# nglaze00/SCoNe_GCN

Hardware: NVIDIA B200
Metric: SCoNe train trajectories/sec (higher is better)
Workload: dtype f32

## Files before the change

### __graft_entry__.py

```python
import os
import shutil
import subprocess
import sys

ROOT = os.path.dirname(os.path.abspath(__file__))
SRC = ['scone_gcn_b200/csrc/scone_complex.cu', 'scone_gcn_b200/csrc/scone_kernels.cu', 'scone_gcn_b200/csrc/scone_model.cu',
       'scone_gcn_b200/csrc/scone_bunch.cu', 'scone_gcn_b200/csrc/scone_slab.cu', 'scone_gcn_b200/csrc/scone_rows.cu',
       'scone_gcn_b200/csrc/scone_fused.cu', 'scone_gcn_b200/csrc/scone_plan_table.cu', 'scone_gcn_b200/csrc/scone_umma.cu',
       'scone_gcn_b200/csrc/scone_dp.cu']
OUT = 'scone_gcn_b200/libscone_b200.so'
NVCC_FLAGS = ['-O3', '-std=c++17', '-gencode', 'arch=compute_100a,code=sm_100a', '-lineinfo', '-Xcompiler', '-fPIC',
              '-Iinclude']
OBJ_DIR = 'build/obj'


def _stale(out, deps):
    if not os.path.exists(out):
        return True
    t = os.path.getmtime(out)
    return any(os.path.getmtime(d) > t for d in deps)


def build(force=False):
    os.chdir(ROOT)
    deps = SRC + ['include/scone_b200.h', 'scone_gcn_b200/csrc/common.cuh', 'scone_gcn_b200/csrc/slab_common.cuh', 'scone_gcn_b200/csrc/fused.cuh']
    hdrs = ['include/scone_b200.h', 'scone_gcn_b200/csrc/common.cuh', 'scone_gcn_b200/csrc/slab_common.cuh', 'scone_gcn_b200/csrc/fused.cuh']
    if force or _stale(OUT, deps):
        nvcc = shutil.which('nvcc') or '/usr/local/cuda/bin/nvcc'
        os.makedirs(OBJ_DIR, exist_ok=True)
        objs, procs = [], []
        for src in SRC:
            obj = os.path.join(OBJ_DIR, os.path.basename(src)[:-3] + '.o')
            objs.append(obj)
            if force or _stale(obj, [src] + hdrs):
                cmd = [nvcc] + NVCC_FLAGS + ['-c', '-o', obj, src]
                print('[build]', ' '.join(cmd), flush=True)
                procs.append((cmd, subprocess.Popen(cmd)))
        for cmd, p in procs:
            if p.wait() != 0:
                raise subprocess.CalledProcessError(p.returncode, cmd)
        cmd = [nvcc, '-shared', '-gencode', 'arch=compute_100a,code=sm_100a', '-o', OUT] + objs
        print('[build]', ' '.join(cmd), flush=True)
        subprocess.check_call(cmd)
    _build_xla_ffi_shim(force)
    if ROOT not in sys.path:
        sys.path.insert(0, ROOT)
    import scone_gcn_b200
    L = scone_gcn_b200.lib()
    assert L.scone_version() == 100
    print('[build] ok:', scone_gcn_b200.library_path())


def _build_xla_ffi_shim(force=False):
    src, out = 'scone_gcn_b200/csrc/scone_xla_ffi.cc', 'scone_gcn_b200/libscone_b200_xla.so'
    inc = None
    try:
        import jaxlib
        cand = os.path.join(os.path.dirname(jaxlib.__file__), 'include')
        if os.path.exists(os.path.join(cand, 'xla', 'ffi', 'api', 'ffi.h')):
            inc = cand
    except Exception:
        pass
    cxx = shutil.which('g++') or 'g++'
    if inc is None:
        os.makedirs(OBJ_DIR, exist_ok=True)
        subprocess.check_call([cxx, '-std=c++17', '-Iinclude', '-c', '-o', os.path.join(OBJ_DIR, 'scone_xla_ffi.o'), src])
        print('[build] jax FFI shim skipped (jaxlib / xla/ffi/api/ffi.h not found); %s compile-checked' % src, flush=True)
        return
    if force or _stale(out, [src, 'include/scone_b200.h', OUT]):
        cuda_inc = os.path.join(os.environ.get('CUDA_HOME', '/usr/local/cuda'), 'include')
        cmd = [cxx, '-std=c++17', '-O2', '-shared', '-fPIC', '-Iinclude', '-I' + inc, '-I' + cuda_inc, '-o', out, src,
               '-Lscone_gcn_b200', '-lscone_b200', '-Wl,-rpath,$ORIGIN']
        print('[build]', ' '.join(cmd), flush=True)
        subprocess.check_call(cmd)


def smoke():
    os.chdir(ROOT)
    for p in (ROOT, os.path.join(ROOT, 'tests')):
        if p not in sys.path:
            sys.path.insert(0, p)
    import numpy as np
    import torch
    assert torch.cuda.is_available(), 'smoke() needs a CUDA device'
    torch.cuda.set_device(0)
    import scone_gcn_b200 as sg
    from golden_util import Dataset
    from oracle import scone_oracle as so
    ds = Dataset('dataset_small.npz')
    cx = sg.SimplicialComplex.from_simplices(ds.N, ds.edges, ds.faces, 'scone')
    net = sg.SconeModel(cx, [16, 16, 16], micro_batch=32)
    rs = np.random.RandomState(0)
    W = [0.3 * rs.randn(*s) for s in net.shapes]
    net.set_weights(W)
    ptr, fe, fv = sg.flows_to_csr(ds.flows)
    lp = net.forward(ptr, fe, fv, ds.last_nodes)
    orc = so.DenseOracle('scone', so.shift_matrices(ds.B1, ds.B2, 'scone'), ds.B1, ds.last_nodes, ds.flows, ds.targets)
    with torch.no_grad():
        ref = orc.forward(W).numpy()[:, :, 0]
    err = float(np.abs(lp - ref).max())
    assert err < 1e-5 * max(1.0, float(np.abs(ref).max())), 'log-prob mismatch vs oracle: %g' % err
    mask = ds.train_mask.astype(np.float32)
    buf = net.loss_grad(ptr, fe, fv, ds.last_nodes, ds.raw['targets_argmax'], mask)
    l_ref, g_ref = orc.loss_and_grads(W, ds.train_mask, 0.0)
    n = net.n_params
    g = net.unflatten(buf[:n] / buf[n + 1])
    gerr = max(float(np.abs(a - b).max() / max(np.abs(b).max(), 1e-30)) for a, b in zip(g, g_ref))
    assert abs(buf[n] / buf[n + 1] - l_ref) < 1e-5 * max(1.0, abs(float(l_ref))) and gerr < 1e-4, (buf[n] / buf[n + 1], l_ref, gerr)
    net.adam_step(0, 1e-3, 5e-5)
    torch.cuda.synchronize()
    print('[smoke] ok: max |dlogp| = %.2e, max rel grad err = %.2e, launches = %d'
          % (err, gerr, sg.lib().scone_launch_count()))


if __name__ == '__main__':
    {'build': build, 'smoke': smoke}[sys.argv[1] if len(sys.argv) > 1 else 'build']()
```

### scone_gcn_b200/csrc/scone_fused.cu

```cuda
#include <algorithm>
#include <cstdlib>
#include <cub/device/device_radix_sort.cuh>
#include "common.cuh"
#include "fused.cuh"

namespace {

#include "slab_common.cuh"

constexpr int kTrajThreads = 256;
constexpr int kFuMaxD = SCONE_MAX_DEGREE;
constexpr uint32_t kNoRow = 0xFFFFu;
constexpr uint32_t kFlaggedKey = 0xFFFFFFu;

template <int ACT>
__device__ __forceinline__ float fu_act(float z) {
    if (ACT == SCONE_ACT_TANH) return scone_tanh(z);
    if (ACT == SCONE_ACT_LEAKY_RELU) return z >= 0.f ? z : 0.01f * z;
    return fmaxf(z, 0.f);
}
template <int ACT>
__device__ __forceinline__ float fu_dact(float h) {
    if (ACT == SCONE_ACT_TANH) return 1.f - h * h;
    if (ACT == SCONE_ACT_LEAKY_RELU) return h >= 0.f ? 1.f : 0.01f;
    return h > 0.f ? 1.f : 0.f;
}

__device__ __forceinline__ int align2(int x) { return (x + 1) & ~1; }

struct EdgeSet {
    int* keys;
    int mask, shift;
    __device__ __forceinline__ unsigned home(int e) const { return ((unsigned)e * 2654435761u) >> shift; }
    __device__ __forceinline__ int insert(int e, bool& is_new) {
        unsigned h = home(e);
        is_new = false;
        for (int probes = 0; probes <= mask; ++probes) {
            const int old = atomicCAS(&keys[h], -1, e);
            if (old == -1) {
                is_new = true;
                return (int)h;
            }
            if (old == e) return (int)h;
            h = (h + 1) & mask;
        }
        return -1;
    }
    __device__ __forceinline__ int find(int e) const {
        unsigned h = home(e);
        int k = keys[h];
        while (k != e) {
            if (k == -1) return -1;
            h = (h + 1) & mask;
            k = keys[h];
        }
        return (int)h;
    }
};

struct FuPairs {
    int s_ptr[kFuMaxD], s_off[kFuMaxD + 1];
    __device__ __forceinline__ int setup(const int32_t* __restrict__ nbrhoods, const int32_t* __restrict__ inc_ptr, int last, bool last_ok, int D) {
        for (int j = threadIdx.x; j < D; j += blockDim.x) {
            const int nbr = last_ok ? nbrhoods[(size_t)last * D + j] : -1;
            s_ptr[j] = nbr >= 0 ? inc_ptr[nbr] : -1;
            s_off[j + 1] = nbr >= 0 ? inc_ptr[nbr + 1] - inc_ptr[nbr] : 0;
        }
        __syncthreads();
        if (threadIdx.x == 0) {
            s_off[0] = 0;
            for (int j = 0; j < D; ++j) s_off[j + 1] += s_off[j];
        }
        __syncthreads();
        return s_off[D];
    }
    __device__ __forceinline__ int slot_of(int i, int D) const {
        int j = 0;
        while (j + 1 < D && s_off[j + 1] <= i) ++j;
        return j;
    }
};

template <int THREADS>
__device__ __forceinline__ void plan_trajectory(const PlanArgs& a, const int t, unsigned char* sm) {
    constexpr int QUADS = THREADS / 4;
    const int HS = a.HS, LV = a.LV, EC = a.EC, L = a.L, D = a.D;
    int* keys = reinterpret_cast<int*>(sm);
    float* xv = reinterpret_cast<float*>(keys + HS);
    int* lvl = reinterpret_cast<int*>(xv + HS);
    uint16_t* idx0 = reinterpret_cast<uint16_t*>(lvl + HS);
    int* rowcnt = reinterpret_cast<int*>(idx0 + 3 * HS);
    int* erow = rowcnt + LV + 4;
    int* live_edge = erow + LV + 4;
    uint16_t* live = reinterpret_cast<uint16_t*>(live_edge + LV);
    uint16_t* rankA = live + LV;
    uint16_t* rankB = rankA + LV;
    uint16_t* ebuf = rankB + LV;
    __shared__ FuPairs pairs;
    __shared__ int s_nhash, s_nlive, s_ovf, s_warp[THREADS / 32];
    __shared__ unsigned s_piece;

    const int tid = threadIdx.x, lane = tid & 31, ql = tid & 3;
    const unsigned qmask = 0xFu << (lane & ~3);
    int* hdr = a.hdr + (size_t)t * kFusedHdrW;
    auto give_up = [&]() {
        if (tid == 0) {
            if (a.retry != nullptr) {
                hdr[0] = kFusedFlagRetry;
                a.retry[atomicAdd(a.n_retry, 1)] = t;
            } else {
                hdr[0] = kFusedFlagOverflow;
                *a.overflow = 1;
            }
        }
    };
    for (int i = tid; i < HS; i += THREADS) {
        keys[i] = -1;
        xv[i] = 0.f;
        lvl[i] = 0;
    }
    for (int i = tid; i < 3 * HS; i += THREADS) idx0[i] = (uint16_t)kNoRow;
    if (tid == 0) s_nhash = s_ovf = s_nlive = 0;
    const int last = a.last_nodes[t];
    const bool last_ok = last >= 0 && last < a.N;
    const int total_pairs = pairs.setup(a.nbrhoods, a.inc_ptr, last, last_ok, D);
    EdgeSet set{keys, HS - 1, a.hshift};
    const int hash_cap = (HS * 3) / 4;
    auto alloc = [&](int words) -> unsigned {
        __syncthreads();
        if (tid == 0) {
            const unsigned long long w = (unsigned long long)align2(words);
            const unsigned long long o = atomicAdd(a.bump, w);
            if (o + w > a.arena_words) {
                s_ovf = 2;
                s_piece = 0u;
            } else {
                s_piece = (unsigned)o;
            }
        }
        __syncthreads();
        return s_piece;
    };
    const int fp0 = a.traj_ptr[t], fp1 = a.traj_ptr[t + 1];

    {
        const unsigned c0 = last_ok ? a.cone_ptr[last] : 0u, c1 = last_ok ? a.cone_ptr[last + 1] : 0u;
        const int n_cone = (int)(c1 - c0);
        if (n_cone > hash_cap) {
            give_up();
            return;
        }
        for (int i = tid; i < n_cone; i += THREADS) {
            const uint32_t en = a.cone_ent[c0 + i];
            bool is_new;
            const int s = set.insert((int)(en & 0x3FFFFFFFu), is_new);
            lvl[s] = (int)(en >> 30);
        }
        if (tid == 0) s_nhash = n_cone;
    }
    __syncthreads();
    for (int p = fp0 + tid; p < fp1; p += THREADS) {
        const int eo = a.flow_edge[p];
        if (eo < 0 || eo >= a.E) continue;
        const int s = set.find(a.rank[eo]);
        if (s >= 0) xv[s] = a.flow_val[p];
    }
    __syncthreads();
    auto mark = [&](int s2, int l) {
        const int bit = 1 << (8 + l);
        const int old = atomicOr(&lvl[s2], bit);
        if (!(old & bit)) {
            const int k = atomicAdd(&s_nlive, 1);
            if (k < LV) {
                live[k] = (uint16_t)s2;
                live_edge[k] = keys[s2];
            } else {
                s_ovf = 1;
            }
        }
    };
    auto rank_live = [&](uint16_t* idx, uint16_t* byrank) -> int {
        __syncthreads();
        const int n = min(s_nlive, LV);
        for (int k = tid; k < n; k += THREADS) {
            const int e = live_edge[k];
            int r = 0;
            for (int m = 0; m < n; ++m) r += live_edge[m] < e ? 1 : 0;
            idx[live[k]] = (uint16_t)r;
            byrank[r] = live[k];
        }
        __syncthreads();
        return n;
    };

    for (int p = fp0 + (tid >> 2); p < fp1; p += QUADS) {
        const int eo = a.flow_edge[p];
        if (eo < 0 || eo >= a.E) continue;
        const int e = a.rank[eo];
        const int s = set.find(e);
        if (s < 0 || xv[s] == 0.f) continue;
        const int p1 = a.mptr[e + 1];
        for (int q = a.mptr[e] + ql; q < p1; q += 4) {
            const int s2 = set.find(a.ment[q].x);
            if (s2 >= 0 && (lvl[s2] & 0xFF) >= 1) mark(s2, 1);
        }
    }
    uint16_t *rcur = rankA, *rnext = rankB;
    int n_cur = rank_live(idx0 + 1 * HS, rcur);
    if (s_ovf) {
        give_up();
        return;
    }
    int n_l[kFusedMaxL + 1] = {0, 0, 0, 0};
    unsigned off_l1 = 0, off_f[kFusedMaxL + 1] = {0, 0, 0, 0}, off_b[kFusedMaxL + 1] = {0, 0, 0, 0};
    int tot_f[kFusedMaxL + 1] = {0, 0, 0, 0}, tot_b[kFusedMaxL + 1] = {0, 0, 0, 0};

    auto emit_program = [&](const uint16_t* byrank, int n_rows, const uint16_t* idx, int& total_out) -> unsigned {
        for (int r = tid >> 2; r < n_rows; r += QUADS) {
            const int b0 = erow[r], b1 = erow[r + 1];
            int c = 0;
            for (int i = b0 + ql; i < b1; i += 4) {
                const uint32_t s2 = ebuf[i];
                if (s2 != kNoRow && idx[s2] != (uint16_t)kNoRow) ++c;
            }
            c += __shfl_xor_sync(qmask, c, 1);
            c += __shfl_xor_sync(qmask, c, 2);
            if (ql == 0) rowcnt[r] = c;
        }
        __syncthreads();
        const int total = fused_block_scan_excl<THREADS>(rowcnt, n_rows, s_warp);
        total_out = total;
        const unsigned off = alloc(align2(n_rows + 1) + 2 * total);
        if (!s_ovf) {
            int* pdst = reinterpret_cast<int*>(a.arena + off);
            int2* edst = reinterpret_cast<int2*>(a.arena + off + align2(n_rows + 1));
            for (int r = tid; r <= n_rows; r += THREADS) pdst[r] = rowcnt[r];
            for (int r = tid >> 2; r < n_rows; r += QUADS) {
                const int e = keys[byrank[r]];
                const int p0 = a.mptr[e], b0 = erow[r], b1 = erow[r + 1];
                int base = rowcnt[r];
                for (int i0 = b0; i0 < b1; i0 += 4) {
                    const int i = i0 + ql;
                    uint32_t rr = kNoRow;
                    if (i < b1) {
                        const uint32_t s2 = ebuf[i];
                        if (s2 != kNoRow) rr = idx[s2];
                    }
                    const bool valid = rr != kNoRow;
                    const unsigned bits = (__ballot_sync(qmask, valid) >> (lane & ~3)) & 0xFu;
                    if (valid) {
                        const int2 en = a.ment[p0 + (i - b0)];
                        edst[base + __popc(bits & ((1u << ql) - 1u))] = make_int2((int)(rr | (en.x == e ? 0x80000000u : 0u)), en.y);
                    }
                    base += __popc(bits);
                }
            }
        }
        __syncthreads();
        return off;
    };

    for (int l = 1; l <= L; ++l) {
        uint16_t* idx_prev = idx0 + ((l + 2) % 3) * HS;
        uint16_t* idx_next = idx0 + ((l + 1) % 3) * HS;
        n_l[l] = n_cur;
        for (int r = tid; r < n_cur; r += THREADS) {
            const int e = keys[rcur[r]];
            rowcnt[r] = a.mptr[e + 1] - a.mptr[e];
        }
        __syncthreads();
        const int n_ent = fused_block_scan_excl<THREADS>(rowcnt, n_cur, s_warp);
        if (n_ent > EC) {
            if (tid == 0) s_ovf = 1;
            __syncthreads();
            break;
        }
        for (int r = tid; r <= n_cur; r += THREADS) erow[r] = rowcnt[r];
        __syncthreads();
        for (int r = tid >> 2; r < n_cur; r += QUADS) {
            const int e = keys[rcur[r]];
            const int p0 = a.mptr[e], b0 = erow[r], len = erow[r + 1] - b0;
            for (int i = ql; i < len; i += 4) {
                const int s2 = set.find(a.ment[p0 + i].x);
                ebuf[b0 + i] = s2 >= 0 ? (uint16_t)s2 : (uint16_t)kNoRow;
            }
        }
        __syncthreads();
        if (l == 1) {
            off_l1 = alloc(3 * n_cur);
            if (!s_ovf) {
                float* dst = reinterpret_cast<float*>(a.arena + off_l1);
                for (int r = tid >> 2; r < n_cur; r += QUADS) {
                    const int slot = rcur[r];
                    const int e = keys[slot];
                    const int p0 = a.mptr[e], b0 = erow[r], len = erow[r + 1] - b0;
                    float a1 = 0.f, a2 = 0.f;
                    for (int i = ql; i < len; i += 4) {
                        const uint32_t s2 = ebuf[b0 + i];
                        const float x = s2 != kNoRow ? xv[s2] : 0.f;
                        if (x != 0.f) {
                            const int pk = a.ment[p0 + i].y;
                            a1 = fmaf((float)(short)(pk & 0xffff), x, a1);
                            a2 = fmaf((float)(pk >> 16), x, a2);
                        }
                    }
#pragma unroll
                    for (int o = 1; o < 4; o <<= 1) {
                        a1 += __shfl_xor_sync(qmask, a1, o);
                        a2 += __shfl_xor_sync(qmask, a2, o);
                    }
                    if (ql == 0) {
                        dst[3 * r + 0] = xv[slot];
                        dst[3 * r + 1] = a1;
                        dst[3 * r + 2] = a2;
                    }
                }
            }
            __syncthreads();
        } else {
            off_f[l] = emit_program(rcur, n_cur, idx_prev, tot_f[l]);
        }
        if (l == L) break;
        if (tid == 0) s_nlive = 0;
        for (int i = tid; i < HS; i += THREADS) idx_next[i] = (uint16_t)kNoRow;
        __syncthreads();
        for (int i = tid; i < n_ent; i += THREADS) {
            const uint32_t s2 = ebuf[i];
            if (s2 != kNoRow && (lvl[s2] & 0xFF) >= l + 1) mark((int)s2, l + 1);
        }
        const int n_next = rank_live(idx_next, rnext);
        if (s_ovf) break;
        off_b[l + 1] = emit_program(rcur, n_cur, idx_next, tot_b[l + 1]);
        uint16_t* tmp = rcur; rcur = rnext; rnext = tmp;
        n_cur = n_next;
    }
    __syncthreads();
    if (s_ovf == 1) {
        give_up();
        return;
    }
    const uint16_t* idxL = idx0 + (L % 3) * HS;
    const unsigned off_ro = alloc(align2(D + 1) + 2 * total_pairs);
    if (!s_ovf) {
        int* pdst = reinterpret_cast<int*>(a.arena + off_ro);
        int2* edst = reinterpret_cast<int2*>(a.arena + off_ro + align2(D + 1));
        for (int j = tid; j <= D; j += THREADS) pdst[j] = pairs.s_off[j];
        for (int i = tid; i < total_pairs; i += THREADS) {
            const int j = pairs.slot_of(i, D);
            const int2 es = a.inc_ent[pairs.s_ptr[j] + (i - pairs.s_off[j])];
            const int s = set.find(es.x);
            const uint32_t r = s >= 0 ? (uint32_t)idxL[s] : kNoRow;
            edst[i] = make_int2((int)(r | ((uint32_t)j << 16)), es.y);
        }
    }
    __syncthreads();
    if (s_ovf) {
        if (tid == 0) {
            hdr[0] = kFusedFlagOverflow;
            *a.overflow = 1;
        }
        return;
    }
    if (tid == 0) {
        hdr[0] = 0;
        for (int l = 1; l <= kFusedMaxL; ++l) hdr[l] = l <= L ? n_l[l] : 0;
        hdr[4] = (int)off_l1;
        for (int l = 2; l <= kFusedMaxL; ++l) {
            hdr[5 + (l - 2)] = (int)off_f[l];
            hdr[7 + (l - 2)] = (int)off_b[l];
        }
        hdr[9] = (int)off_ro;
        hdr[10] = total_pairs;
        hdr[11] = s_nhash;
        hdr[12] = tot_f[2];
        hdr[13] = fp1 - fp0;
        hdr[14] = tot_f[3];
        hdr[15] = min(tot_b[2], 0xFFFF) | (min(tot_b[3], 0xFFFF) << 16);
    }
}

template <int THREADS>
__global__ void __launch_bounds__(THREADS) fused_plan_kernel(const PlanArgs a) {
    extern __shared__ __align__(16) unsigned char sm[];
    const int n_work = a.tier == 0 ? a.n_work : *a.n_in;
    for (int w = blockIdx.x; w < n_work; w += gridDim.x) {
        plan_trajectory<THREADS>(a, a.tier == 0 ? w : a.in_list[w], sm);
        __syncthreads();
    }
}

struct TrajArgs {
    const int* hdr;
    const uint32_t* arena;
    const int32_t* rows;
    const uint32_t* okeys;
    const int32_t* order;
    const float* W;
    int w_off[3 * kFusedMaxL + 1];
    int L, b, D, n_params;
    float* logprobs;
    const int32_t* target_idx;
    const float* mask;
    float* partial;
    float* scratch;
    size_t scratch_stride;
    int cap_rows;
    int big_rows;
    unsigned long long* rows_done;
};

template <int C>
struct FuGeom {
    static constexpr int LDH = C + 8;
    static constexpr int LDA = 3 * C + 4;
    static constexpr int LDW = C + 8;
    static constexpr int CH = 80;
    static constexpr int SE = 1024;
    static constexpr int SP = 200;
    static constexpr int SL1 = 384;
    static constexpr int LPR = C / 4;
    static constexpr int NP = C / 16;
    static constexpr int NMT = C / 16;
    static constexpr int NNT = 3 * C / 8;
    static constexpr int WPM = 8 / NMT;
    static constexpr int TPW = (NNT + WPM - 1) / WPM;
};

template <int C>
__device__ __forceinline__ void fu_gather(float* __restrict__ tile, const float* src, const int* ptr, const int2* ent, int pbase, int nr) {
    using G = FuGeom<C>;
    const int lr = threadIdx.x % G::LPR, rr = threadIdx.x / G::LPR;
    const int npad = (nr + 15) & ~15;
    for (int r = rr; r < npad; r += kTrajThreads / G::LPR) {
        u64 s0a = 0ull, s0b = 0ull, s1a = 0ull, s1b = 0ull;
        int own = -1;
        if (r < nr) {
            const int p1 = ptr[r + 1] - pbase;
            for (int p = ptr[r] - pbase; p < p1; ++p) {
                const int2 en = ent[p];
                const float c0 = (float)(short)(en.y & 0xffff), c1 = (float)(en.y >> 16);
                const float* vp = src + (size_t)(en.x & 0xFFFF) * G::LDH + 4 * lr;
                const ulonglong2 v = *reinterpret_cast<const ulonglong2*>(vp);
                const u64 q0 = bcast2(c0), q1 = bcast2(c1);
                ffma2(s0a, q0, v.x);
                ffma2(s0b, q0, v.y);
                ffma2(s1a, q1, v.x);
                ffma2(s1b, q1, v.y);
                own = en.x < 0 ? (en.x & 0xFFFF) : own;
            }
        }
        float4 o = make_float4(0.f, 0.f, 0.f, 0.f);
        if (own >= 0) o = *reinterpret_cast<const float4*>(src + (size_t)own * G::LDH + 4 * lr);
        float* d = tile + (size_t)r * G::LDA + 4 * lr;
        *reinterpret_cast<float4*>(d) = o;
        *reinterpret_cast<ulonglong2*>(d + C) = make_ulonglong2(s0a, s0b);
        *reinterpret_cast<ulonglong2*>(d + 2 * C) = make_ulonglong2(s1a, s1b);
    }
}

__device__ __forceinline__ void cp_async_4(void* dst, const void* src) {
    asm volatile("cp.async.ca.shared.global [%0], [%1], 4;" ::"r"((unsigned)__cvta_generic_to_shared(dst)), "l"(src) : "memory");
}
__device__ __forceinline__ void cp_async_8(void* dst, const void* src) {
    asm volatile("cp.async.ca.shared.global [%0], [%1], 8;" ::"r"((unsigned)__cvta_generic_to_shared(dst)), "l"(src) : "memory");
}
__device__ __forceinline__ void cp_async_wait_all() { asm volatile("cp.async.wait_all;" ::: "memory"); }

template <int C>
__device__ __forceinline__ bool fu_prefetch(const uint32_t* __restrict__ arena, unsigned off, int n_rows, int tot, int* sptr, int2* sent) {
    using G = FuGeom<C>;
    if (n_rows + 1 > G::SP || tot > G::SE) return false;
    const int* gptr = reinterpret_cast<const int*>(arena + off);
    const int2* gent = reinterpret_cast<const int2*>(gptr + align2(n_rows + 1));
    for (int i = threadIdx.x; i <= n_rows; i += kTrajThreads) cp_async_4(sptr + i, gptr + i);
    for (int i = threadIdx.x; i < tot; i += kTrajThreads) cp_async_8(sent + i, gent + i);
    return true;
}

template <int C>
__device__ __forceinline__ int fu_stage(const int* __restrict__ gptr, const int2* __restrict__ gent, int r0, int n_rows, int* sptr,
                                        int2* sent, bool* staged) {
    using G = FuGeom<C>;
    int nr = min(G::CH, n_rows - r0);
    for (int i = threadIdx.x; i <= nr; i += kTrajThreads) sptr[i] = __ldg(gptr + r0 + i);
    __syncthreads();
    const int pbase = sptr[0];
    while (nr > 16 && sptr[nr] - pbase > G::SE) nr -= 16;
    const int cnt = sptr[nr] - pbase;
    *staged = cnt <= G::SE;
    if (*staged)
        for (int i = threadIdx.x; i < cnt; i += kTrajThreads) sent[i] = __ldg(gent + pbase + i);
    __syncthreads();
    return nr;
}

template <int C, bool TRANSPOSED, typename Epi>
__device__ __forceinline__ void fu_product(const float* __restrict__ tile, const float* __restrict__ Wsm, int nr, Epi epi) {
    using G = FuGeom<C>;
    const int lane = threadIdx.x & 31, warp = threadIdx.x >> 5, g = lane >> 2, tig = lane & 3;
    const int n_mt = (nr + 15) >> 4;
    for (int tl = warp; tl < n_mt * G::NP; tl += kTrajThreads / 32) {
        const int mt = tl / G::NP, np = tl % G::NP;
        float d[2][4], dx[2][4];
#pragma unroll
        for (int j = 0; j < 2; ++j)
#pragma unroll
            for (int q = 0; q < 4; ++q) d[j][q] = dx[j][q] = 0.f;
        const float* arow0 = tile + (size_t)(16 * mt + g) * G::LDA + tig;
        const float* arow1 = arow0 + 8 * G::LDA;
#pragma unroll 4
        for (int ks = 0; ks < 3 * C / 8; ++ks) {
            const int k0 = 8 * ks;
            uint32_t ahi[4], alo[4];
            split_tf32(arow0[k0], ahi[0], alo[0]);
            split_tf32(arow1[k0], ahi[1], alo[1]);
            split_tf32(arow0[k0 + 4], ahi[2], alo[2]);
            split_tf32(arow1[k0 + 4], ahi[3], alo[3]);
#pragma unroll
            for (int j = 0; j < 2; ++j) {
                const int n0 = (2 * np + j) * 8;
                float b0, b1;
                if (!TRANSPOSED) {
                    b0 = Wsm[(k0 + tig) * G::LDW + n0 + g];
                    b1 = Wsm[(k0 + tig + 4) * G::LDW + n0 + g];
                } else {
                    const int term = k0 / C, co = k0 % C + tig;
                    b0 = Wsm[(term * C + n0 + g) * G::LDW + co];
                    b1 = Wsm[(term * C + n0 + g) * G::LDW + co + 4];
                }
                uint32_t bh0, bl0, bh1, bl1;
                split_tf32(b0, bh0, bl0);
                split_tf32(b1, bh1, bl1);
                mma_tf32(dx[j], alo, bh0, bh1);
                mma_tf32(dx[j], ahi, bl0, bl1);
                mma_tf32(d[j], ahi, bh0, bh1);
            }
        }
#pragma unroll
        for (int j = 0; j < 2; ++j)
#pragma unroll
            for (int q = 0; q < 4; ++q) d[j][q] += dx[j][q];
#pragma unroll
        for (int j = 0; j < 2; ++j) {
            const int col = (2 * np + j) * 8 + 2 * tig;
            const int r0 = 16 * mt + g, r1 = r0 + 8;
            if (r0 < nr) epi(r0, col, d[j][0], d[j][1]);
            if (r1 < nr) epi(r1, col, d[j][2], d[j][3]);
        }
    }
}

template <int C>
__device__ __forceinline__ void fu_dw(float (&acc)[FuGeom<C>::TPW][4], const float* hprev, const float* __restrict__ tile, int nr) {
    using G = FuGeom<C>;
    const int lane = threadIdx.x & 31, warp = threadIdx.x >> 5, g = lane >> 2, tig = lane & 3;
    const int mt = warp % G::NMT, ntg = warp / G::NMT;
    for (int k0 = 0; k0 < nr; k0 += 8) {
        const int ra = k0 + tig, rb = ra + 4;
        const float* ha = hprev + (size_t)ra * G::LDH + 16 * mt + g;
        const float* hb = hprev + (size_t)rb * G::LDH + 16 * mt + g;
        uint32_t ahi[4], alo[4];
        split_tf32(ra < nr ? ha[0] : 0.f, ahi[0], alo[0]);
        split_tf32(ra < nr ? ha[8] : 0.f, ahi[1], alo[1]);
        split_tf32(rb < nr ? hb[0] : 0.f, ahi[2], alo[2]);
        split_tf32(rb < nr ? hb[8] : 0.f, ahi[3], alo[3]);
#pragma unroll
        for (int s = 0; s < G::TPW; ++s) {
            const int nt = ntg + G::WPM * s;
            if (nt < G::NNT) {
                uint32_t bh0, bl0, bh1, bl1;
                split_tf32(tile[(size_t)ra * G::LDA + 8 * nt + g], bh0, bl0);
                split_tf32(tile[(size_t)rb * G::LDA + 8 * nt + g], bh1, bl1);
                mma_tf32(acc[s], alo, bh0, bh1);
                mma_tf32(acc[s], ahi, bl0, bl1);
                mma_tf32(acc[s], ahi, bh0, bh1);
            }
        }
    }
}

template <int C, int ACT, bool GRAD, bool BIG>
__global__ void __launch_bounds__(kTrajThreads, 2) fused_traj_kernel(const TrajArgs a) {
    using G = FuGeom<C>;
    extern __shared__ __align__(16) unsigned char sm[];
    const int L = a.L, D = a.D;
    float* Wsm = reinterpret_cast<float*>(sm);
    float* w1s = Wsm + (size_t)(kFusedMaxL - 1) * 3 * C * G::LDW;
    float* wos = w1s + 3 * C;
    float* tile = wos + C;
    float* zs = tile + (size_t)G::CH * G::LDA;
    float* lg = zs + (size_t)D * C;
    float* dl = lg + ((D + 3) & ~3);
    int2* sent = reinterpret_cast<int2*>(dl + ((D + 3) & ~3));
    int* sptr = reinterpret_cast<int*>(sent + G::SE);
    float* l1s = reinterpret_cast<float*>(sptr + G::SP);
    float* rows_sm = l1s + 2 * G::SL1;
    const int tid = threadIdx.x, lane = tid & 31, warp = tid >> 5;

    for (int l = 2; l <= L; ++l)
        for (int i = tid; i < 3 * C * C; i += kTrajThreads) {
            const int term = i / (C * C), rem = i % (C * C);
            Wsm[(size_t)(l - 2) * 3 * C * G::LDW + (term * C + rem / C) * G::LDW + rem % C] = a.W[a.w_off[3 * (l - 1) + term] + rem];
        }
    for (int i = tid; i < 3 * C; i += kTrajThreads) w1s[i] = a.W[a.w_off[i / C] + i % C];
    for (int i = tid; i < C; i += kTrajThreads) wos[i] = a.W[a.w_off[3 * L] + i];
    __syncthreads();

    float acc[kFusedMaxL - 1][G::TPW][4];
#pragma unroll
    for (int l = 0; l < kFusedMaxL - 1; ++l)
#pragma unroll
        for (int s = 0; s < G::TPW; ++s)
#pragma unroll
            for (int q = 0; q < 4; ++q) acc[l][s][q] = 0.f;
    float acc1 = 0.f, acc_out = 0.f, acc_nll = 0.f, acc_cnt = 0.f;
    unsigned long long n_fwd = 0, n_bwd = 0;

    float* rows = BIG ? a.scratch + (size_t)blockIdx.x * a.scratch_stride : rows_sm;

    __shared__ int s_range[2];
    __shared__ int s_hdr[2][kFusedHdrW];
    if (tid == 0) {
        int f = 0, hi = a.b;
        while (f < hi) {
            const int mid = (f + hi) >> 1;
            if (a.okeys[mid] >= kFlaggedKey) f = mid + 1;
            else hi = mid;
        }
        int lo = f;
        hi = a.b;
        while (lo < hi) {
            const int mid = (lo + hi) >> 1;
            if ((int)a.okeys[mid] > a.cap_rows) lo = mid + 1;
            else hi = mid;
        }
        s_range[0] = BIG ? f : lo;
        s_range[1] = BIG ? lo : a.b;
    }
    __syncthreads();
    const int i_lo = s_range[0], i_hi = s_range[1];
    auto index_of = [&](int kk) { return i_lo + kk * (int)gridDim.x + ((kk & 1) ? (int)gridDim.x - 1 - (int)blockIdx.x : (int)blockIdx.x); };
    auto issue_first = [&](const int* hn, float* l1buf) -> bool {
        const int n1 = hn[1];
        if (3 * n1 <= G::SL1) {
            const float* l1g = reinterpret_cast<const float*>(a.arena + (unsigned)hn[4]);
            for (int i = tid; i < 3 * n1; i += kTrajThreads) cp_async_4(l1buf + i, l1g + i);
        }
        return L >= 2 ? fu_prefetch<C>(a.arena, (unsigned)hn[5], hn[2], hn[12], sptr, sent)
                      : fu_prefetch<C>(a.arena, (unsigned)hn[9], D, hn[10], sptr, sent);
    };
    bool have = index_of(0) < i_hi, pf_first = false;
    int t = 0;
    if (have) {
        t = a.order[index_of(0)];
        const int rid = a.rows != nullptr ? a.rows[t] : t;
        if (tid < kFusedHdrW) s_hdr[0][tid] = a.hdr[(size_t)rid * kFusedHdrW + tid];
        __syncthreads();
        pf_first = issue_first(s_hdr[0], l1s);
    }
    for (int k = 0; have; ++k) {
        const int* h = s_hdr[k & 1];
        float* l1buf = l1s + (k & 1) * G::SL1;
        const bool have_next = index_of(k + 1) < i_hi;
        const int t_next = have_next ? a.order[index_of(k + 1)] : 0;
        bool issued_next = false, pf_first_next = false;
        cp_async_wait_all();
        __syncthreads();
        int n[kFusedMaxL + 1], hb[kFusedMaxL + 2];
        int tot = 0;
        n[0] = 0;
        hb[0] = hb[1] = 0;
#pragma unroll
        for (int l = 1; l <= kFusedMaxL; ++l) {
            n[l] = l <= L ? h[l] : 0;
            hb[l] = tot;
            tot += n[l];
        }
        const float* l1 = reinterpret_cast<const float*>(a.arena + (unsigned)h[4]);
        n_fwd += (unsigned long long)tot;
        const int tot_f[kFusedMaxL + 1] = {0, 0, h[12], h[14]};
        const int tot_b[kFusedMaxL + 1] = {0, 0, h[15] & 0xFFFF, (int)((unsigned)h[15] >> 16)};
        bool pf = pf_first;
        if (3 * n[1] <= G::SL1) l1 = l1buf;

        for (int i = tid; i < n[1] * C; i += kTrajThreads) {
            const int r = i / C, c = i % C;
            const float z = fmaf(l1[3 * r + 2], w1s[2 * C + c], fmaf(l1[3 * r + 1], w1s[C + c], l1[3 * r] * w1s[c]));
            rows[(size_t)r * G::LDH + c] = fu_act<ACT>(z);
        }
        const int rid_next = have_next ? (a.rows != nullptr ? a.rows[t_next] : t_next) : 0;
        __syncthreads();
#pragma unroll
        for (int l = 2; l <= kFusedMaxL; ++l) {
            if (l > L) break;
            const int nl = n[l];
            const int* ptr = reinterpret_cast<const int*>(a.arena + (unsigned)h[5 + (l - 2)]);
            const int2* ent = reinterpret_cast<const int2*>(ptr + align2(nl + 1));
            const float* hprev = rows + (size_t)hb[l - 1] * G::LDH;
            float* hout = rows + (size_t)hb[l] * G::LDH;
            const float* Wl = Wsm + (size_t)(l - 2) * 3 * C * G::LDW;
            bool pf_next = false;
            if (nl == 0)
                pf_next = l < L ? fu_prefetch<C>(a.arena, (unsigned)h[5 + (l - 1)], n[l + 1], tot_f[l < kFusedMaxL ? l + 1 : l], sptr, sent)
                                : fu_prefetch<C>(a.arena, (unsigned)h[9], D, h[10], sptr, sent);
            for (int r0 = 0; r0 < nl;) {
                int nr;
                if (pf) {
                    nr = min(G::CH, nl - r0);
                    fu_gather<C>(tile, hprev, sptr + r0, sent, 0, nr);
                } else {
                    bool staged;
                    nr = fu_stage<C>(ptr, ent, r0, nl, sptr, sent, &staged);
                    if (staged) fu_gather<C>(tile, hprev, sptr, sent, sptr[0], nr);
                    else fu_gather<C>(tile, hprev, sptr, ent, 0, nr);
                }
                __syncthreads();
                if (r0 + nr >= nl)
                    pf_next = l < L ? fu_prefetch<C>(a.arena, (unsigned)h[5 + (l - 1)], n[l + 1], tot_f[l < kFusedMaxL ? l + 1 : l], sptr, sent)
                                    : fu_prefetch<C>(a.arena, (unsigned)h[9], D, h[10], sptr, sent);
                fu_product<C, false>(tile, Wl, nr, [&](int r, int col, float v0, float v1) {
                    float* o = hout + (size_t)(r0 + r) * G::LDH + col;
                    *reinterpret_cast<float2*>(o) = make_float2(fu_act<ACT>(v0), fu_act<ACT>(v1));
                });
                cp_async_wait_all();
                __syncthreads();
                r0 += nr;
            }
            if (nl == 0) {
                cp_async_wait_all();
                __syncthreads();
            }
            pf = pf_next;
        }
        if (have_next && tid < kFusedHdrW) cp_async_4(&s_hdr[(k + 1) & 1][tid], a.hdr + (size_t)rid_next * kFusedHdrW + tid);
        const int* rptr = reinterpret_cast<const int*>(a.arena + (unsigned)h[9]);
        const int2* rent = reinterpret_cast<const int2*>(rptr + align2(D + 1));
        if (pf) {
            rptr = sptr;
            rent = sent;
        } else if (h[10] <= G::SE) {
            for (int i = tid; i <= D; i += kTrajThreads) sptr[i] = __ldg(rptr + i);
            for (int i = tid; i < h[10]; i += kTrajThreads) sent[i] = __ldg(rent + i);
            __syncthreads();
            rptr = sptr;
            rent = sent;
        }
        const float* hL = rows + (size_t)hb[L] * G::LDH;
        for (int j = warp; j < D; j += kTrajThreads / 32) {
            float z = 0.f;
            const int p1 = rptr[j + 1];
            for (int p = rptr[j]; p < p1; ++p) {
                const int2 en = rent[p];
                const uint32_t r = (uint32_t)en.x & 0xFFFFu;
                if (r != kNoRow && lane < C) z = fmaf(__int_as_float(en.y), hL[(size_t)r * G::LDH + lane], z);
            }
            if (lane < C) zs[j * C + lane] = z;
            float part = lane < C ? z * wos[lane] : 0.f;
#pragma unroll
            for (int o = 16; o > 0; o >>= 1) part += __shfl_xor_sync(0xffffffffu, part, o);
            if (lane == 0) lg[j] = part;
        }
        __syncthreads();
        if (warp == 0) {
            float mx = -3.4e38f;
            for (int j = lane; j < D; j += 32) mx = fmaxf(mx, lg[j]);
#pragma unroll
            for (int o = 16; o > 0; o >>= 1) mx = fmaxf(mx, __shfl_xor_sync(0xffffffffu, mx, o));
            float se = 0.f;
            for (int j = lane; j < D; j += 32) se += expf(lg[j] - mx);
#pragma unroll
            for (int o = 16; o > 0; o >>= 1) se += __shfl_xor_sync(0xffffffffu, se, o);
            const float lse = mx + logf(se);
            const float mk = GRAD ? a.mask[t] : 0.f;
            const int y = GRAD ? a.target_idx[t] : -1;
            for (int j = lane; j < D; j += 32) {
                const float lp = lg[j] - lse;
                if (a.logprobs != nullptr) a.logprobs[(size_t)t * D + j] = lp;
                if (GRAD) {
                    dl[j] = mk * (expf(lp) - (j == y ? 1.f : 0.f));
                    if (j == y) acc_nll += -mk * lp;
                }
            }
            if (GRAD && lane == 0) acc_cnt += mk;
        }
        if (!GRAD) {
            cp_async_wait_all();
            __syncthreads();
            if (have_next) pf_first = issue_first(s_hdr[(k + 1) & 1], l1s + ((k + 1) & 1) * G::SL1);
            t = t_next;
            have = have_next;
            continue;
        }
        const int nL = n[L];
        float* gL = rows + (size_t)hb[L] * G::LDH;
        for (int r = tid; r < nL; r += kTrajThreads) gL[(size_t)r * G::LDH + C] = 0.f;
        __syncthreads();
        if (tid < C) {
            float s = acc_out;
            for (int j = 0; j < D; ++j) s = fmaf(dl[j], zs[j * C + tid], s);
            acc_out = s;
        }
        {
            const int npairs = rptr[D];
            for (int p = tid; p < npairs; p += kTrajThreads) {
                const int2 en = rent[p];
                const uint32_t r = (uint32_t)en.x & 0xFFFFu;
                if (r != kNoRow) atomicAdd(&gL[(size_t)r * G::LDH + C], __int_as_float(en.y) * dl[((uint32_t)en.x >> 16) & 0x7FFFu]);
            }
        }
        __syncthreads();
        pf = L >= 2 ? fu_prefetch<C>(a.arena, (unsigned)h[7 + (L - 2)], n[L - 1], tot_b[L], sptr, sent) : false;
        for (int i = tid; i < nL * C; i += kTrajThreads) {
            const int r = i / C, c = i % C;
            gL[(size_t)r * G::LDH + c] = gL[(size_t)r * G::LDH + C] * wos[c] * fu_dact<ACT>(hL[(size_t)r * G::LDH + c]);
        }
        cp_async_wait_all();
        __syncthreads();
#pragma unroll
        for (int l = kFusedMaxL; l >= 2; --l) {
            if (l > L) continue;
            const int np_ = n[l - 1];
            const int* ptr = reinterpret_cast<const int*>(a.arena + (unsigned)h[7 + (l - 2)]);
            const int2* ent = reinterpret_cast<const int2*>(ptr + align2(np_ + 1));
            const float* gl = rows + (size_t)hb[l] * G::LDH;
            float* hprev = rows + (size_t)hb[l - 1] * G::LDH;
            float* gprev = hprev;
            const float* Wl = Wsm + (size_t)(l - 2) * 3 * C * G::LDW;
            n_bwd += (unsigned long long)np_;
            bool pf_next = false;
            if (np_ == 0 && l > 2) pf_next = fu_prefetch<C>(a.arena, (unsigned)h[7 + (l - 3)], n[l - 2], tot_b[l - 1], sptr, sent);
            for (int r0 = 0; r0 < np_;) {
                int nr;
                if (pf) {
                    nr = min(G::CH, np_ - r0);
                    fu_gather<C>(tile, gl, sptr + r0, sent, 0, nr);
                } else {
                    bool staged;
                    nr = fu_stage<C>(ptr, ent, r0, np_, sptr, sent, &staged);
                    if (staged) fu_gather<C>(tile, gl, sptr, sent, sptr[0], nr);
                    else fu_gather<C>(tile, gl, sptr, ent, 0, nr);
                }
                __syncthreads();
                if (r0 + nr >= np_) {
                    if (l > 2) {
                        pf_next = fu_prefetch<C>(a.arena, (unsigned)h[7 + (l - 3)], n[l - 2], tot_b[l - 1], sptr, sent);
                    } else if (have_next) {
                        pf_first_next = issue_first(s_hdr[(k + 1) & 1], l1s + ((k + 1) & 1) * G::SL1);
                        issued_next = true;
                    }
                }
                fu_dw<C>(acc[l - 2], hprev + (size_t)r0 * G::LDH, tile, nr);
                __syncthreads();
                fu_product<C, true>(tile, Wl, nr, [&](int r, int col, float v0, float v1) {
                    const float2 hv = *reinterpret_cast<const float2*>(hprev + (size_t)(r0 + r) * G::LDH + col);
                    *reinterpret_cast<float2*>(gprev + (size_t)(r0 + r) * G::LDH + col) =
                        make_float2(v0 * fu_dact<ACT>(hv.x), v1 * fu_dact<ACT>(hv.y));
                });
                cp_async_wait_all();
                __syncthreads();
                r0 += nr;
            }
            if (np_ == 0) {
                cp_async_wait_all();
                __syncthreads();
            }
            pf = pf_next;
        }
        if (tid < 3 * C) {
            const int k = tid / C, c = tid % C;
            const float* g1 = rows;
            float s = acc1;
            for (int r = 0; r < n[1]; ++r) s = fmaf(l1[3 * r + k], g1[(size_t)r * G::LDH + c], s);
            acc1 = s;
        }
        if (have_next && !issued_next) {
            cp_async_wait_all();
            __syncthreads();
            pf_first_next = issue_first(s_hdr[(k + 1) & 1], l1s + ((k + 1) & 1) * G::SL1);
        }
        pf_first = pf_first_next;
        t = t_next;
        have = have_next;
    }

    if (a.rows_done != nullptr && tid == 0 && (n_fwd | n_bwd)) {
        atomicAdd(a.rows_done, n_fwd);
        atomicAdd(a.rows_done + 1, n_bwd);
    }
    if (!GRAD) return;
    float* P = a.partial + (size_t)blockIdx.x * (a.n_params + 2);
    if (tid < 3 * C) P[a.w_off[tid / C] + tid % C] = acc1;
    {
        const int g = lane >> 2, tig = lane & 3;
        const int mt = warp % G::NMT, ntg = warp / G::NMT;
#pragma unroll
        for (int l = 2; l <= kFusedMaxL; ++l) {
            if (l > L) break;
#pragma unroll
            for (int s = 0; s < G::TPW; ++s) {
                const int nt = ntg + G::WPM * s;
                if (nt >= G::NNT) continue;
                const int nn = 8 * nt + 2 * tig, term = nn / C, co = nn % C;
                float* dst = P + a.w_off[3 * (l - 1) + term];
                const int ci = 16 * mt + g;
                dst[ci * C + co] = acc[l - 2][s][0];
                dst[ci * C + co + 1] = acc[l - 2][s][1];
                dst[(ci + 8) * C + co] = acc[l - 2][s][2];
                dst[(ci + 8) * C + co + 1] = acc[l - 2][s][3];
            }
        }
    }
    if (tid < C) P[a.w_off[3 * L] + tid] = acc_out;
    if (warp == 0) {
        float s = acc_nll;
#pragma unroll
        for (int o = 16; o > 0; o >>= 1) s += __shfl_xor_sync(0xffffffffu, s, o);
        if (lane == 0) {
            P[a.n_params] = s;
            P[a.n_params + 1] = acc_cnt;
        }
    }
}

__global__ void __launch_bounds__(256) fused_cost_kernel(const int* __restrict__ hdr, const int32_t* __restrict__ rows, int b, int L,
                                                         uint32_t* __restrict__ keys, int32_t* __restrict__ vals) {
    const int t = blockIdx.x * blockDim.x + threadIdx.x;
    if (t >= b) return;
    const int* h = hdr + (size_t)(rows != nullptr ? rows[t] : t) * kFusedHdrW;
    int tot = 0;
    for (int l = 1; l <= L; ++l) tot += h[l];
    keys[t] = h[0] != 0 ? kFlaggedKey : min((uint32_t)tot, kFlaggedKey - 1u);
    vals[t] = t;
}

__global__ void __launch_bounds__(256) fused_reduce_kernel(const float* __restrict__ partial, int nparts, int n, float* __restrict__ out) {
    __shared__ float red[8][32];
    const int lane = threadIdx.x & 31, warp = threadIdx.x >> 5;
    const int i = blockIdx.x * 32 + lane;
    float s = 0.f;
    if (i < n)
        for (int p = warp; p < nparts; p += 8) s += partial[(size_t)p * n + i];
    red[warp][lane] = s;
    __syncthreads();
    if (warp == 0 && i < n)
        out[i] += ((red[0][lane] + red[1][lane]) + (red[2][lane] + red[3][lane])) + ((red[4][lane] + red[5][lane]) + (red[6][lane] + red[7][lane]));
}

size_t plan_smem_bytes(int HS, int LV, int EC) {
    return (size_t)HS * 18 + (size_t)(LV + 4) * 8 + (size_t)LV * 10 + (size_t)EC * 2 + 16;
}

template <int C>
size_t traj_smem_bytes(int D, int cap_rows) {
    using G = FuGeom<C>;
    size_t fl = (size_t)(kFusedMaxL - 1) * 3 * C * G::LDW + 3 * C + C + (size_t)G::CH * G::LDA + (size_t)D * C + 2 * ((D + 3) & ~3) +
                2 * (size_t)G::SE + G::SP + 2 * G::SL1 + (size_t)cap_rows * G::LDH;
    return fl * sizeof(float);
}

template <int C, int ACT, bool GRAD>
int launch_traj(const TrajArgs& base, int grid_small, int grid_big, size_t smem_small, size_t smem_big, cudaStream_t st) {
    static bool configured = false;
    if (!configured) {
        SCONE_CUDA(cudaFuncSetAttribute(fused_traj_kernel<C, ACT, GRAD, false>, cudaFuncAttributeMaxDynamicSharedMemorySize, 227 * 1024 - 1024));
        SCONE_CUDA(cudaFuncSetAttribute(fused_traj_kernel<C, ACT, GRAD, true>, cudaFuncAttributeMaxDynamicSharedMemorySize, 227 * 1024 - 1024));
        configured = true;
    }
    TrajArgs a = base;
    fused_traj_kernel<C, ACT, GRAD, false><<<grid_small, kTrajThreads, smem_small, st>>>(a);
    SCONE_LAUNCHED();
    if (grid_big > 0) {
        if (GRAD) a.partial = base.partial + (size_t)grid_small * (base.n_params + 2);
        fused_traj_kernel<C, ACT, GRAD, true><<<grid_big, kTrajThreads, smem_big, st>>>(a);
        SCONE_LAUNCHED();
    }
    return 0;
}

template <int C, bool GRAD>
int dispatch_traj(int act, const TrajArgs& a, int gs, int gb, size_t ss, size_t sb, cudaStream_t st) {
    switch (act) {
        case SCONE_ACT_TANH: return launch_traj<C, SCONE_ACT_TANH, GRAD>(a, gs, gb, ss, sb, st);
        case SCONE_ACT_LEAKY_RELU: return launch_traj<C, SCONE_ACT_LEAKY_RELU, GRAD>(a, gs, gb, ss, sb, st);
        case SCONE_ACT_RELU: return launch_traj<C, SCONE_ACT_RELU, GRAD>(a, gs, gb, ss, sb, st);
    }
    scone_set_error("unknown activation %d", act);
    return 2;
}

int run_traj(FusedState* f, int act, TrajArgs& t, float* grad, cudaStream_t st) {
    const bool want_grad = grad != nullptr;
    const int n = t.b;
    if (n > f->sort_cap) {
        cudaFree(f->d_sort);
        cudaFree(f->d_sort_tmp);
        f->d_sort = nullptr;
        f->d_sort_tmp = nullptr;
        f->sort_cap = 0;
        uint32_t* k = nullptr;
        int32_t* v = nullptr;
        size_t bytes = 0;
        SCONE_CUDA(cub::DeviceRadixSort::SortPairsDescending(nullptr, bytes, k, k, v, v, n, 0, 24, st));
        SCONE_CUDA(cudaMalloc((void**)&f->d_sort, 4 * (size_t)n * sizeof(uint32_t)));
        SCONE_CUDA(cudaMalloc((void**)&f->d_sort_tmp, bytes ? bytes : 16));
        f->sort_tmp_bytes = bytes;
        f->sort_cap = n;
    }
    uint32_t* k_in = f->d_sort;
    uint32_t* k_out = k_in + f->sort_cap;
    int32_t* v_in = reinterpret_cast<int32_t*>(k_out + f->sort_cap);
    int32_t* v_out = v_in + f->sort_cap;
    ScopedProf prof(want_grad ? SCONE_K_LAYER_BWD : SCONE_K_LAYER_FWD, st);
    fused_cost_kernel<<<(n + 255) / 256, 256, 0, st>>>(t.hdr, t.rows, n, f->L, k_in, v_in);
    SCONE_LAUNCHED();
    size_t bytes = f->sort_tmp_bytes;
    SCONE_CUDA(cub::DeviceRadixSort::SortPairsDescending(f->d_sort_tmp, bytes, k_in, k_out, v_in, v_out, n, 0, 24, st));
    t.okeys = k_out;
    t.order = v_out;
    int rc;
    if (f->C == 32)
        rc = want_grad ? dispatch_traj<32, true>(act, t, f->grid_small, f->grid_big, f->traj_smem_small, f->traj_smem_big, st)
                       : dispatch_traj<32, false>(act, t, f->grid_small, f->grid_big, f->traj_smem_small, f->traj_smem_big, st);
    else
        rc = want_grad ? dispatch_traj<16, true>(act, t, f->grid_small, f->grid_big, f->traj_smem_small, f->traj_smem_big, st)
                       : dispatch_traj<16, false>(act, t, f->grid_small, f->grid_big, f->traj_smem_small, f->traj_smem_big, st);
    if (rc) return rc;
    if (want_grad) {
        const int np = (int)f->n_params + 2;
        fused_reduce_kernel<<<(np + 31) / 32, 256, 0, st>>>(f->d_partial, f->grid_small + f->grid_big, np, grad);
        SCONE_LAUNCHED();
    }
    return 0;
}

}

bool scone_fused_supported(const scone_complex* cx, int n_layers, const int32_t* hidden) {
    if (cx->d_mptr == nullptr || cx->D > kFuMaxD || cx->D < 1 || n_layers < 1 || n_layers > kFusedMaxL) return false;
    for (int l = 0; l < n_layers; ++l)
        if (hidden[l] != hidden[0] || (hidden[l] != 16 && hidden[l] != 32)) return false;
    return true;
}

void scone_fused_destroy(FusedState* f) {
    if (!f) return;
    cudaFree(f->d_hdr); cudaFree(f->d_retry); cudaFree(f->d_arena); cudaFree(f->d_set_hdr); cudaFree(f->d_set_arena); cudaFree(f->d_set_bump); cudaFree(f->d_bump); cudaFree(f->d_partial); cudaFree(f->d_scratch); cudaFree(f->d_stats);
    cudaFree(f->d_rows_done); cudaFree(f->d_sort); cudaFree(f->d_sort_tmp);
    scone_table_destroy(f);
    delete f;
}

static void table_shape(int entries, int* HS, int* hshift) {
    int hs = 256;
    while (hs * 3 / 4 < entries + 1) hs *= 2;
    *HS = hs;
    *hshift = 32;
    for (int v = hs; v > 1; v >>= 1) --*hshift;
}

int scone_fused_create(const scone_complex* cx, int L, int C, int mb, int64_t n_params, FusedState** out) {
    *out = nullptr;
    if ((unsigned)cx->E >= (1u << 30)) return 0;
    FusedState* f = new FusedState();
    f->L = L;
    f->C = C;
    f->n_params = n_params;
    {
        bool ok = false;
        const int rc = scone_table_build(cx, f, L, &ok);
        if (rc || !ok) {
            scone_fused_destroy(f);
            return rc;
        }
    }
    int max_row = 1;
    {
        std::vector<int32_t> mp((size_t)cx->E + 1);
        SCONE_CUDA(cudaMemcpy(mp.data(), cx->d_mptr, mp.size() * sizeof(int32_t), cudaMemcpyDeviceToHost));
        for (int e = 0; e < cx->E; ++e) max_row = std::max(max_row, mp[e + 1] - mp[e]);
    }
    constexpr int kMaxPlanSmem = 225 * 1024;
    f->LV = (f->bound_list + 63) & ~63;
    table_shape(f->bound_cone, &f->HS, &f->hshift);
    f->EC = (int)std::min<long long>((long long)f->bound_list * max_row, 1ll << 30);
    f->EC = (f->EC + 63) & ~63;
    {
        const size_t fixed = plan_smem_bytes(f->HS, f->LV, 0);
        if (fixed + 2 * (size_t)f->EC > (size_t)kMaxPlanSmem && fixed + 2 * 8192 <= (size_t)kMaxPlanSmem)
            f->EC = (int)(((size_t)kMaxPlanSmem - fixed) / 2) & ~63;
    }
    f->plan_smem = plan_smem_bytes(f->HS, f->LV, f->EC);
    if (!f->tb_rows && (f->plan_smem > (size_t)kMaxPlanSmem || f->bound_list >= 0xFFFF || f->HS > 32768)) {
        scone_fused_destroy(f);
        return 0;
    }
    {
        table_shape(f->quantile_cone, &f->HS0, &f->hshift0);
        f->LV0 = std::min(192, f->LV);
        f->EC0 = std::min(3072, f->EC);
        f->two_tiers = f->HS0 < f->HS || f->LV0 < f->LV || f->EC0 < f->EC;
        if (!f->two_tiers) {
            f->HS0 = f->HS;
            f->hshift0 = f->hshift;
        }
        auto env_int = [](const char* name, int dflt) {
            const char* v = getenv(name);
            return v && *v ? atoi(v) : dflt;
        };
        if (f->two_tiers) {
            const int hs0 = env_int("SCONE_FUSED_HS0", f->HS0);
            if (hs0 != f->HS0 && hs0 >= 256 && hs0 <= f->HS && (hs0 & (hs0 - 1)) == 0) table_shape((hs0 * 3) / 4 - 1, &f->HS0, &f->hshift0);
            f->LV0 = std::min(env_int("SCONE_FUSED_LV0", f->LV0), f->LV);
            f->EC0 = std::min(env_int("SCONE_FUSED_EC0", f->EC0), f->EC);
        }
        f->plan_smem0 = plan_smem_bytes(f->HS0, f->LV0, f->EC0);
    }
    SCONE_CUDA(cudaFuncSetAttribute(fused_plan_kernel<256>, cudaFuncAttributeMaxDynamicSharedMemorySize, kMaxPlanSmem));
    SCONE_CUDA(cudaFuncSetAttribute(fused_plan_kernel<1024>, cudaFuncAttributeMaxDynamicSharedMemorySize, kMaxPlanSmem));
    const int ldh = C + 8;
    f->cap_rows = C == 32 ? 192 : 384;
    f->big_rows = L * f->bound_list;
    f->traj_smem_small = C == 32 ? traj_smem_bytes<32>(cx->D, f->cap_rows) : traj_smem_bytes<16>(cx->D, f->cap_rows);
    f->traj_smem_big = C == 32 ? traj_smem_bytes<32>(cx->D, 0) : traj_smem_bytes<16>(cx->D, 0);
    if (f->traj_smem_small > 113 * 1024) {
        const size_t over = f->traj_smem_small - 113 * 1024;
        const int less = (int)((over + ldh * 4 - 1) / (ldh * 4));
        f->cap_rows = f->cap_rows > less + 32 ? f->cap_rows - less : 32;
        f->traj_smem_small = C == 32 ? traj_smem_bytes<32>(cx->D, f->cap_rows) : traj_smem_bytes<16>(cx->D, f->cap_rows);
    }
    f->grid_small = 2 * cx->num_sms;
    f->grid_big = f->big_rows > f->cap_rows ? 2 * cx->num_sms : 0;
    if (f->grid_big) {
        f->scratch_stride = (size_t)f->big_rows * ldh;
        SCONE_CUDA(cudaMalloc((void**)&f->d_scratch, (size_t)f->grid_big * f->scratch_stride * sizeof(float)));
    }
    SCONE_CUDA(cudaMalloc((void**)&f->d_partial, (size_t)(f->grid_small + f->grid_big) * (n_params + 2) * sizeof(float)));
    const unsigned long long bl = (unsigned long long)f->bound_list;
    unsigned long long worst = 3 * bl + 2 + (unsigned long long)(cx->D + 3) + 2ull * cx->D * cx->D + 16;
    for (int l = 2; l <= L; ++l)
        worst += 2 * (bl + 3) + 4 * bl * (unsigned long long)max_row;
    const unsigned long long budget_words = (1ull << 30) - 1024;
    const unsigned long long share_words = 16 * 1024;
    f->worst_words = worst;
    if (worst * (unsigned long long)mb <= budget_words) {
        f->chunk = mb;
        f->arena_words = worst * (unsigned long long)mb;
    } else {
        f->chunk = (int)std::min<unsigned long long>((unsigned long long)mb, std::max<unsigned long long>(1, budget_words / std::min(worst, share_words)));
        f->arena_words = std::min(budget_words, worst * (unsigned long long)f->chunk);
    }
    SCONE_CUDA(cudaMalloc((void**)&f->d_arena, f->arena_words * sizeof(uint32_t)));
    SCONE_CUDA(cudaMalloc((void**)&f->d_hdr, (size_t)f->chunk * kFusedHdrW * sizeof(int)));
    SCONE_CUDA(cudaMalloc((void**)&f->d_retry, 2 * (size_t)f->chunk * sizeof(int)));
    SCONE_CUDA(cudaMalloc((void**)&f->d_bump, 2 * sizeof(unsigned long long)));
    SCONE_CUDA(cudaMalloc((void**)&f->d_rows_done, 4 * sizeof(unsigned long long)));
    SCONE_CUDA(cudaMemset(f->d_rows_done, 0, 4 * sizeof(unsigned long long)));
    *out = f;
    return 0;
}

static int launch_plans(const scone_complex* cx, const FusedState* f, PlanArgs p, int b, cudaStream_t st) {
    if (f->tb_rows) return scone_table_plan_launch(f, p, b, cx->num_sms, st);
    p.tier = 0; p.n_work = b;
    p.HS = f->HS0; p.LV = f->LV0; p.EC = f->EC0; p.hshift = f->hshift0;
    int* retry = p.retry;
    if (!f->two_tiers) p.retry = nullptr;
    fused_plan_kernel<256><<<b, 256, f->plan_smem0, st>>>(p);
    SCONE_LAUNCHED();
    if (f->two_tiers) {
        p.tier = 1; p.HS = f->HS; p.LV = f->LV; p.EC = f->EC; p.hshift = f->hshift; p.n_in = p.n_retry; p.in_list = retry; p.retry = nullptr;
        fused_plan_kernel<1024><<<std::min(b, cx->num_sms), 1024, f->plan_smem, st>>>(p);
        SCONE_LAUNCHED();
    }
    return 0;
}

int scone_fused_begin(FusedState* f, cudaStream_t st) {
    SCONE_CUDA(cudaMemsetAsync(f->d_bump, 0, 2 * sizeof(unsigned long long), st));
    return 0;
}

static PlanArgs plan_args(const scone_complex* cx, FusedState* f, int off, const int32_t* traj_ptr, const int32_t* flow_edge,
                          const float* flow_val, const int32_t* last_nodes, int* overflow) {
    PlanArgs p{};
    p.traj_ptr = traj_ptr + off; p.flow_edge = flow_edge; p.flow_val = flow_val; p.last_nodes = last_nodes + off;
    p.rank = cx->d_rank; p.nbrhoods = cx->d_nbrhoods; p.inc_ptr = cx->d_inc_ptr; p.inc_ent = cx->d_inc_ent;
    p.mptr = cx->d_mptr; p.ment = cx->d_ment; p.cone_ptr = f->d_cone_ptr; p.cone_ent = f->d_cone_ent;
    p.N = cx->N; p.D = cx->D; p.E = cx->E; p.L = f->L;
    p.hdr = f->d_hdr + (size_t)off * kFusedHdrW; p.arena = f->d_arena; p.bump = f->d_bump; p.arena_words = f->arena_words; p.overflow = overflow;
    p.n_retry = reinterpret_cast<int*>(f->d_bump + 1); p.retry = f->d_retry;
    return p;
}

int scone_fused_plan_part(const scone_complex* cx, FusedState* f, int off, int b, const int32_t* traj_ptr, const int32_t* flow_edge,
                          const float* flow_val, const int32_t* last_nodes, int* overflow, cudaStream_t st, bool defer_tiers) {
    if (b <= 0) return 0;
    SCONE_REQUIRE(off >= 0 && off + b <= f->chunk, "scone_fused_plan_part: trajectories %d .. %d exceed the planned chunk of %d", off, off + b, f->chunk);
    ScopedProf prof(SCONE_K_CONE, st);
    if (defer_tiers && f->tb_rows) {
        PlanArgs p = plan_args(cx, f, 0, traj_ptr, flow_edge, flow_val, last_nodes, overflow);
        p.t0 = off;
        return scone_table_plan_launch(f, p, b, cx->num_sms, st, 0);
    }
    if (off > 0) SCONE_CUDA(cudaMemsetAsync(f->d_bump + 1, 0, sizeof(unsigned long long), st));
    return launch_plans(cx, f, plan_args(cx, f, off, traj_ptr, flow_edge, flow_val, last_nodes, overflow), b, st);
}

int scone_fused_plan_finish(const scone_complex* cx, FusedState* f, int B, const int32_t* traj_ptr, const int32_t* flow_edge,
                            const float* flow_val, const int32_t* last_nodes, int* overflow, cudaStream_t st) {
    if (B <= 0 || !f->tb_rows) return 0;
    ScopedProf prof(SCONE_K_CONE, st);
    return scone_table_plan_launch(f, plan_args(cx, f, 0, traj_ptr, flow_edge, flow_val, last_nodes, overflow), B, cx->num_sms, st, 1);
}

int scone_fused_compute(const scone_complex* cx, FusedState* f, int act, int b, const float* W, const int64_t* w_off, float* logprobs,
                        const int32_t* target_idx, const float* mask, float* grad, bool count_rows, cudaStream_t st) {
    if (b <= 0) return 0;
    TrajArgs t;
    t.hdr = f->d_hdr; t.arena = f->d_arena; t.rows = nullptr; t.W = W;
    for (int i = 0; i <= 3 * kFusedMaxL; ++i) t.w_off[i] = i <= 3 * f->L ? (int)w_off[i] : 0;
    t.L = f->L; t.b = b; t.D = cx->D; t.n_params = (int)f->n_params;
    t.logprobs = logprobs; t.target_idx = target_idx; t.mask = mask;
    t.partial = f->d_partial; t.scratch = f->d_scratch; t.scratch_stride = f->scratch_stride;
    t.cap_rows = f->cap_rows; t.big_rows = f->big_rows;
    t.rows_done = count_rows ? f->d_rows_done : nullptr;
    return run_traj(f, act, t, grad, st);
}

int scone_fused_run(const scone_complex* cx, FusedState* f, int act, int b, const int32_t* traj_ptr, const int32_t* flow_edge,
                    const float* flow_val, const int32_t* last_nodes, const float* W, const int64_t* w_off, float* logprobs,
                    const int32_t* target_idx, const float* mask, float* grad, int* overflow, bool count_rows, cudaStream_t st) {
    if (b <= 0) return 0;
    SCONE_REQUIRE(b <= f->chunk, "scone_fused_run: chunk of %d trajectories exceeds the planned %d", b, f->chunk);
    int rc = scone_fused_begin(f, st);
    if (!rc) rc = scone_fused_plan_part(cx, f, 0, b, traj_ptr, flow_edge, flow_val, last_nodes, overflow, st);
    if (!rc) rc = scone_fused_compute(cx, f, act, b, W, w_off, logprobs, target_idx, mask, grad, count_rows, st);
    return rc;
}

int scone_fused_plan_set(const scone_complex* cx, FusedState* f, int B, const int32_t* traj_ptr, const int32_t* flow_edge,
                         const float* flow_val, const int32_t* last_nodes, int* overflow, cudaStream_t st) {
    if (B > f->set_cap) {
        cudaFree(f->d_set_hdr);
        cudaFree(f->d_set_arena);
        f->d_set_hdr = nullptr;
        f->d_set_arena = nullptr;
        f->set_cap = 0;
        const unsigned long long budget_words = (1ull << 30) - 1024;
        f->set_arena_words = std::min(budget_words, f->worst_words * (unsigned long long)B);
        SCONE_CUDA(cudaMalloc((void**)&f->d_set_hdr, (size_t)B * kFusedHdrW * sizeof(int)));
        SCONE_CUDA(cudaMalloc((void**)&f->d_set_arena, f->set_arena_words * sizeof(uint32_t)));
        if (!f->d_set_bump) SCONE_CUDA(cudaMalloc((void**)&f->d_set_bump, 2 * sizeof(unsigned long long)));
        f->set_cap = B;
    }
    f->set_n = 0;
    SCONE_CUDA(cudaMemsetAsync(f->d_set_bump, 0, 2 * sizeof(unsigned long long), st));
    PlanArgs p{};
    p.flow_edge = flow_edge; p.flow_val = flow_val;
    p.rank = cx->d_rank; p.nbrhoods = cx->d_nbrhoods; p.inc_ptr = cx->d_inc_ptr; p.inc_ent = cx->d_inc_ent;
    p.mptr = cx->d_mptr; p.ment = cx->d_ment; p.cone_ptr = f->d_cone_ptr; p.cone_ent = f->d_cone_ent;
    p.N = cx->N; p.D = cx->D; p.E = cx->E; p.L = f->L;
    p.arena = f->d_set_arena; p.bump = f->d_set_bump; p.arena_words = f->set_arena_words; p.overflow = overflow;
    p.n_retry = reinterpret_cast<int*>(f->d_set_bump + 1); p.retry = f->d_retry;
    ScopedProf prof(SCONE_K_CONE, st);
    for (int off = 0; off < B; off += f->chunk) {
        const int b = std::min(f->chunk, B - off);
        SCONE_CUDA(cudaMemsetAsync(f->d_set_bump + 1, 0, sizeof(unsigned long long), st));
        p.traj_ptr = traj_ptr + off; p.last_nodes = last_nodes + off; p.hdr = f->d_set_hdr + (size_t)off * kFusedHdrW;
        const int rc = launch_plans(cx, f, p, b, st);
        if (rc) return rc;
    }
    f->set_n = B;
    return 0;
}

int scone_fused_run_planned(const scone_complex* cx, FusedState* f, int act, int n, const int32_t* rows_dev, const float* W, const int64_t* w_off,
                            float* logprobs, const int32_t* target_idx, const float* mask, float* grad, bool count_rows, cudaStream_t st) {
    if (n <= 0) return 0;
    SCONE_REQUIRE(f->set_n > 0, "scone_fused_run_planned: no planned set (call scone_model_plan_* first)");
    SCONE_REQUIRE(rows_dev != nullptr || n <= f->set_n, "scone_fused_run_planned: %d trajectories requested, the planned set holds %d", n, f->set_n);
    TrajArgs t;
    t.hdr = f->d_set_hdr; t.arena = f->d_set_arena; t.rows = rows_dev; t.W = W;
    for (int i = 0; i <= 3 * kFusedMaxL; ++i) t.w_off[i] = i <= 3 * f->L ? (int)w_off[i] : 0;
    t.L = f->L; t.b = n; t.D = cx->D; t.n_params = (int)f->n_params;
    t.logprobs = logprobs; t.target_idx = target_idx; t.mask = mask;
    t.partial = f->d_partial; t.scratch = f->d_scratch; t.scratch_stride = f->scratch_stride;
    t.cap_rows = f->cap_rows; t.big_rows = f->big_rows;
    t.rows_done = count_rows ? f->d_rows_done : nullptr;
    return run_traj(f, act, t, grad, st);
}

int scone_fused_last_retries(FusedState* f) {
    unsigned long long v[2] = {0, 0};
    if (cudaDeviceSynchronize() != cudaSuccess) return -1;
    if (cudaMemcpy(v, f->d_bump, sizeof(v), cudaMemcpyDeviceToHost) != cudaSuccess) return -1;
    return (int)(v[1] & 0xffffffffull);
}

int scone_fused_read(FusedState* f, int t, int* hdr_out, unsigned off, int words, uint32_t* arena_out) {
    SCONE_CUDA(cudaDeviceSynchronize());
    if (hdr_out) SCONE_CUDA(cudaMemcpy(hdr_out, f->d_hdr + (size_t)t * kFusedHdrW, kFusedHdrW * sizeof(int), cudaMemcpyDeviceToHost));
    if (arena_out && words > 0) SCONE_CUDA(cudaMemcpy(arena_out, f->d_arena + off, (size_t)words * sizeof(uint32_t), cudaMemcpyDeviceToHost));
    return 0;
}
```

### scone_gcn_b200/csrc/scone_umma.cu

```cuda
#include <cstdlib>
#include <cstring>
#include "common.cuh"

namespace {

#include "slab_common.cuh"

constexpr int kGatherWarps = 16, kGroupWarps = 8, kUmmaThreads = kGatherWarps * 32;
constexpr int kC = 32;
constexpr int kGatherDepth = 4;
constexpr uint32_t kTmemCols = 512;
constexpr uint32_t kColsAhi = 0, kColsAlo = 96, kColsD = 192, kColsGroup = 224;
constexpr uint32_t kIdesc = (1u << 4) | (2u << 7) | (2u << 10) | ((32u >> 3) << 17) | ((128u >> 4) << 24);
constexpr uint32_t kLbo = 512, kSbo = 128;
constexpr int kSpinLimit = 4000000;

__device__ __forceinline__ uint32_t smem_u32(const void* p) { return (uint32_t)__cvta_generic_to_shared(p); }
__device__ __forceinline__ void tc_fence_before() { asm volatile("tcgen05.fence::before_thread_sync;" ::: "memory"); }
__device__ __forceinline__ void tc_fence_after() { asm volatile("tcgen05.fence::after_thread_sync;" ::: "memory"); }
__device__ __forceinline__ void tc_st_16x128b_x2(uint32_t taddr, uint32_t r0, uint32_t r1, uint32_t r2, uint32_t r3) {
    asm volatile("tcgen05.st.sync.aligned.16x128b.x2.b32 [%0], {%1, %2, %3, %4};" ::"r"(taddr), "r"(r0), "r"(r1), "r"(r2), "r"(r3) : "memory");
}
__device__ __forceinline__ void tc_ld_16x256b_x4(uint32_t taddr, float (&d)[4][4]) {
    uint32_t r[16];
    asm volatile("tcgen05.ld.sync.aligned.16x256b.x4.b32 {%0, %1, %2, %3, %4, %5, %6, %7, %8, %9, %10, %11, %12, %13, %14, %15}, [%16];"
                 : "=r"(r[0]), "=r"(r[1]), "=r"(r[2]), "=r"(r[3]), "=r"(r[4]), "=r"(r[5]), "=r"(r[6]), "=r"(r[7]), "=r"(r[8]), "=r"(r[9]),
                   "=r"(r[10]), "=r"(r[11]), "=r"(r[12]), "=r"(r[13]), "=r"(r[14]), "=r"(r[15])
                 : "r"(taddr)
                 : "memory");
    asm volatile("tcgen05.wait::ld.sync.aligned;" ::: "memory");
#pragma unroll
    for (int nt = 0; nt < 4; ++nt)
#pragma unroll
        for (int q = 0; q < 4; ++q) d[nt][q] = __uint_as_float(r[4 * nt + q]);
}
__device__ __forceinline__ void mbar_init(uint64_t* bar, uint32_t count) {
    asm volatile("mbarrier.init.shared::cta.b64 [%0], %1;" ::"r"(smem_u32(bar)), "r"(count));
}
__device__ __forceinline__ bool mbar_try_wait(uint64_t* bar, uint32_t parity) {
    uint32_t ok;
    asm volatile("{\n\t.reg .pred p;\n\tmbarrier.try_wait.parity.shared::cta.b64 p, [%1], %2;\n\tselp.b32 %0, 1, 0, p;\n\t}"
                 : "=r"(ok)
                 : "r"(smem_u32(bar)), "r"(parity)
                 : "memory");
    return ok != 0;
}
__device__ __forceinline__ void mbar_wait(uint64_t* bar, uint32_t parity, int* err) {
    int spins = 0;
    while (!mbar_try_wait(bar, parity)) {
        if (++spins > kSpinLimit) {
            *err = 1;
            break;
        }
    }
}
__device__ __forceinline__ void umma_commit(uint64_t* bar) {
    asm volatile("tcgen05.commit.cta_group::1.mbarrier::arrive::one.shared::cluster.b64 [%0];" ::"r"(smem_u32(bar)) : "memory");
}
__device__ __forceinline__ void umma_tf32_ts(uint32_t tmem_d, uint32_t tmem_a, uint64_t desc_b, uint32_t accumulate) {
    asm volatile(
        "{\n\t.reg .pred p;\n\tsetp.ne.b32 p, %4, 0;\n\t"
        "tcgen05.mma.cta_group::1.kind::tf32 [%0], [%1], %2, %3, {%5, %5, %5, %5}, p;\n\t}"
        ::"r"(tmem_d), "r"(tmem_a), "l"(desc_b), "r"(kIdesc), "r"(accumulate), "r"(0u)
        : "memory");
}
__device__ __forceinline__ uint64_t umma_desc(uint32_t saddr) {
    return (uint64_t)((saddr >> 4) & 0x3FFF) | ((uint64_t)((kLbo >> 4) & 0x3FFF) << 16) | ((uint64_t)((kSbo >> 4) & 0x3FFF) << 32) |
           ((uint64_t)1 << 46);
}

template <int ACT>
__global__ void __launch_bounds__(kUmmaThreads, 1) layer_fwd_umma_kernel(const float* __restrict__ Hin, float* __restrict__ Hout,
                                                                        const float* __restrict__ W0, const float* __restrict__ W1,
                                                                        const float* __restrict__ W2, const int32_t* __restrict__ mptr,
                                                                        const int2* __restrict__ ment, int E, int b, int chunk, int* __restrict__ err) {
    constexpr int TS = 16;
    using G = SlabGeom<kC, TS>;
    constexpr int NT = kC / 8;
    __shared__ __align__(128) float Bs[2][24 * 4 * 32];
    __shared__ __align__(8) uint64_t s_dfull[2];
    __shared__ unsigned s_arrived[2];
    __shared__ uint32_t s_tmem;
    const int warp = threadIdx.x >> 5, lane = threadIdx.x & 31, tig = lane & 3;

    if (warp == 0) {
        asm volatile("tcgen05.alloc.cta_group::1.sync.aligned.shared::cta.b32 [%0], %1;" ::"r"(smem_u32(&s_tmem)), "r"(kTmemCols));
        asm volatile("tcgen05.relinquish_alloc_permit.cta_group::1.sync.aligned;");
    }
    if (threadIdx.x == 0) {
        s_arrived[0] = s_arrived[1] = 0u;
        mbar_init(&s_dfull[0], 1);
        mbar_init(&s_dfull[1], 1);
    }
    for (int i = threadIdx.x; i < 96 * kC; i += kUmmaThreads) {
        const int k = i / kC, n = i % kC;
        const int term = k / 32, s = (k % 32) / 8, kappa = k % 8;
        const float* W = term == 0 ? W0 : (term == 1 ? W1 : W2);
        const float w = W[G::chan(s, kappa) * kC + n];
        const uint32_t hi = to_tf32(w), lo = to_tf32(w - __uint_as_float(hi));
        const int off = (k / 4) * 128 + (n / 8) * 32 + (n % 8) * 4 + (k % 4);
        Bs[0][off] = __uint_as_float(hi);
        Bs[1][off] = __uint_as_float(lo);
    }
    asm volatile("fence.proxy.async.shared::cta;" ::: "memory");
    asm volatile("fence.mbarrier_init.release.cluster;" ::: "memory");
    tc_fence_before();
    __syncthreads();
    tc_fence_after();

    const int n_ts = (b + TS - 1) / TS;
    const int tiles_per_ts = (E + kGatherWarps - 1) / kGatherWarps;
    const long long n_tiles = (long long)n_ts * tiles_per_ts;
    const long long per = (n_tiles + gridDim.x - 1) / gridDim.x;
    const long long cl = chunk > 0 ? (long long)chunk : per;

    {
        const int group = warp / kGroupWarps, gw = warp % kGroupWarps;
        const uint32_t tbase = s_tmem + (uint32_t)group * kColsGroup;
        const uint32_t lane_base = (uint32_t)(32 * (gw & 3) + 16 * (gw >> 2)) << 16;
        const unsigned rowbytes_in = (unsigned)b * kC * 4u;
        const size_t rowlen_out = (size_t)b * kC;
        uint32_t phase = 0;
        int pe0 = 0, pt0 = 0;
        bool pending = false, plive = false;
        for (long long k = 0;; ++k) {
            const long long tile = ((k / cl) * gridDim.x + blockIdx.x) * cl + k % cl;
            const bool have = tile < n_tiles;
            int e0 = 0, t0 = 0;
            bool live = false;
            u64 acc[3][G::NL][2];
            if (have) {
                const int ts = (int)(tile / tiles_per_ts);
                e0 = (int)(tile - (long long)ts * tiles_per_ts) * kGatherWarps + warp;
                t0 = ts * TS;
                live = e0 < E;
                if (live) {
                    slab_gather<kC, TS, kGatherDepth>(Hin, rowbytes_in, mptr, ment, E, b, e0, t0, acc);
                } else {
#pragma unroll
                    for (int k = 0; k < 3; ++k)
#pragma unroll
                        for (int i = 0; i < G::NL; ++i) acc[k][i][0] = acc[k][i][1] = 0ull;
                }
            }
            if (pending) {
                mbar_wait(&s_dfull[group], phase, err);
                phase ^= 1u;
                tc_fence_after();
                float d[NT][4];
                tc_ld_16x256b_x4(tbase + kColsD + lane_base, d);
                if (plive) {
                    slab_activate<ACT, NT>(d);
#pragma unroll
                    for (int r = 0; r < 2; ++r) {
                        int e, t;
                        slab_row<kC, TS>(r, pe0, pt0, e, t);
                        if (e < E && t < b) {
                            float* dst = Hout + (size_t)e * rowlen_out + (size_t)t * kC + 2 * tig;
#pragma unroll
                            for (int nt = 0; nt < NT; ++nt)
                                *reinterpret_cast<float2*>(dst + nt * 8) = make_float2(d[nt][2 * r], d[nt][2 * r + 1]);
                        }
                    }
                }
            }
            if (have) {
#pragma unroll
                for (int term = 0; term < 3; ++term) {
                    float fr[G::KS][4];
                    slab_fragments<kC, TS>(acc[term], fr);
#pragma unroll
                    for (int s = 0; s < G::KS; ++s) {
                        uint32_t ah[4], al[4];
#pragma unroll
                        for (int q = 0; q < 4; ++q) split_tf32(fr[s][q], ah[q], al[q]);
                        const uint32_t col = (uint32_t)(32 * term + 8 * s);
                        tc_st_16x128b_x2(tbase + kColsAhi + col + lane_base, ah[0], ah[1], ah[2], ah[3]);
                        tc_st_16x128b_x2(tbase + kColsAlo + col + lane_base, al[0], al[1], al[2], al[3]);
                    }
                }
                asm volatile("tcgen05.wait::st.sync.aligned;" ::: "memory");
                tc_fence_before();
                __syncwarp();
                unsigned last_one = 0u;
                if (lane == 0) {
                    unsigned old;
                    asm volatile("atom.acq_rel.cta.shared::cta.add.u32 %0, [%1], 1;" : "=r"(old) : "r"(smem_u32(&s_arrived[group])) : "memory");
                    last_one = (old % kGroupWarps) == (unsigned)(kGroupWarps - 1) ? 1u : 0u;
                    if (last_one) {
                        tc_fence_after();
                        const uint32_t bhi = smem_u32(&Bs[0][0]), blo = smem_u32(&Bs[1][0]);
#pragma unroll
                        for (int j = 0; j < 12; ++j) {
                            const uint64_t dh = umma_desc(bhi + (uint32_t)j * 2 * kLbo), dl = umma_desc(blo + (uint32_t)j * 2 * kLbo);
                            umma_tf32_ts(tbase + kColsD, tbase + kColsAlo + 8 * j, dh, j > 0 ? 1u : 0u);
                            umma_tf32_ts(tbase + kColsD, tbase + kColsAhi + 8 * j, dl, 1u);
                            umma_tf32_ts(tbase + kColsD, tbase + kColsAhi + 8 * j, dh, 1u);
                        }
                        umma_commit(&s_dfull[group]);
                    }
                }
                __syncwarp();
                pending = true;
                plive = live;
                pe0 = e0;
                pt0 = t0;
            } else {
                break;
            }
        }
    }
    tc_fence_before();
    __syncthreads();
    if (warp == 0) asm volatile("tcgen05.dealloc.cta_group::1.sync.aligned.b32 %0, %1;" ::"r"(s_tmem), "r"(kTmemCols));
}

int* g_umma_err = nullptr;

int g_dense_chunk = -1;
int scone_dense_chunk() {
    int& chunk = g_dense_chunk;
    if (chunk < 0) {
        const char* e = getenv("SCONE_DENSE_CHUNK");
        chunk = e ? atoi(e) : 8;
        if (chunk < 0) chunk = 0;
    }
    return chunk;
}

constexpr int kFlushTiles = 32;
constexpr int kDW = 3 * kC * kC;

template <int NW>
struct BwdBuf {
    static constexpr uint32_t SBO_A = 128u;
    static constexpr uint32_t LBO_A = 1600u;
    static constexpr uint32_t A_BYTES = 4u * LBO_A;
    static constexpr uint32_t SBO_B = 128u;
    static constexpr uint32_t LBO_B = 528u;
    static constexpr uint32_t B_BYTES = 4u * LBO_B;
    static constexpr uint32_t WARP_BYTES = 2u * A_BYTES + 2u * B_BYTES;
};
constexpr uint32_t kBwdBfBytes = 3u * 4u * 4u * 32u * 16u;

__device__ __forceinline__ uint64_t umma_desc2(uint32_t saddr, uint32_t lbo, uint32_t sbo) {
    return (uint64_t)((saddr >> 4) & 0x3FFF) | ((uint64_t)((lbo >> 4) & 0x3FFF) << 16) | ((uint64_t)((sbo >> 4) & 0x3FFF) << 32) |
           ((uint64_t)1 << 46);
}
__device__ __forceinline__ void umma_tf32_ss(uint32_t tmem_d, uint64_t desc_a, uint64_t desc_b, uint32_t accumulate) {
    asm volatile(
        "{\n\t.reg .pred p;\n\tsetp.ne.b32 p, %4, 0;\n\t"
        "tcgen05.mma.cta_group::1.kind::tf32 [%0], %1, %2, %3, {%5, %5, %5, %5}, p;\n\t}"
        ::"r"(tmem_d), "l"(desc_a), "l"(desc_b), "r"(kIdesc), "r"(accumulate), "r"(0u)
        : "memory");
}
__device__ __forceinline__ void tc_ld_32x32b_x32(uint32_t taddr, uint32_t (&r)[32]) {
    asm volatile(
        "tcgen05.ld.sync.aligned.32x32b.x32.b32 {%0, %1, %2, %3, %4, %5, %6, %7, %8, %9, %10, %11, %12, %13, %14, %15, %16, %17, %18, "
        "%19, %20, %21, %22, %23, %24, %25, %26, %27, %28, %29, %30, %31}, [%32];"
        : "=r"(r[0]), "=r"(r[1]), "=r"(r[2]), "=r"(r[3]), "=r"(r[4]), "=r"(r[5]), "=r"(r[6]), "=r"(r[7]), "=r"(r[8]), "=r"(r[9]),
          "=r"(r[10]), "=r"(r[11]), "=r"(r[12]), "=r"(r[13]), "=r"(r[14]), "=r"(r[15]), "=r"(r[16]), "=r"(r[17]), "=r"(r[18]),
          "=r"(r[19]), "=r"(r[20]), "=r"(r[21]), "=r"(r[22]), "=r"(r[23]), "=r"(r[24]), "=r"(r[25]), "=r"(r[26]), "=r"(r[27]),
          "=r"(r[28]), "=r"(r[29]), "=r"(r[30]), "=r"(r[31])
        : "r"(taddr)
        : "memory");
    asm volatile("tcgen05.wait::ld.sync.aligned;" ::: "memory");
}

template <int ACT>
__device__ __forceinline__ float umma_dact(float h) {
    if (ACT == SCONE_ACT_TANH) return 1.f - h * h;
    if (ACT == SCONE_ACT_LEAKY_RELU) return h >= 0.f ? 1.f : 0.01f;
    return h > 0.f ? 1.f : 0.f;
}

template <int ACT, bool WG, int NW, int DEPTH>
__global__ void __launch_bounds__(NW * 32, 1) layer_bwd_umma_kernel(const float* __restrict__ Gd, const float* Hin, float* Gprev,
                                                                       const float* __restrict__ W0, const float* __restrict__ W1,
                                                                       const float* __restrict__ W2, float* __restrict__ ws,
                                                                       const int32_t* __restrict__ mptr, const int2* __restrict__ ment,
                                                                       int E, int b, int interleave, int* __restrict__ err) {
    constexpr int TS = 16;
    using G = SlabGeom<kC, TS>;
    using L = BwdBuf<NW>;
    constexpr int NT = kC / 8;
    extern __shared__ __align__(128) unsigned char bw_smem[];
    __shared__ __align__(8) uint64_t s_bar[NW];
    __shared__ int s_used[NW];
    __shared__ uint32_t s_tmem;
    const int warp = threadIdx.x >> 5, lane = threadIdx.x & 31, tig = lane & 3, g = lane >> 2;
    uint4* Bf = reinterpret_cast<uint4*>(bw_smem);

    if (warp == 0) {
        asm volatile("tcgen05.alloc.cta_group::1.sync.aligned.shared::cta.b32 [%0], %1;" ::"r"(smem_u32(&s_tmem)), "r"(kTmemCols));
        asm volatile("tcgen05.relinquish_alloc_permit.cta_group::1.sync.aligned;");
    }
    if (threadIdx.x < NW) {
        mbar_init(&s_bar[threadIdx.x], 1);
        s_used[threadIdx.x] = 0;
    }
    if (WG) stage_weight_fragments<kC, kC, TS, true>(Bf, W0, W1, W2);
    asm volatile("fence.mbarrier_init.release.cluster;" ::: "memory");
    tc_fence_before();
    __syncthreads();
    tc_fence_after();

    const uint32_t a_hi = smem_u32(bw_smem) + kBwdBfBytes + (uint32_t)warp * L::WARP_BYTES, a_lo = a_hi + L::A_BYTES;
    const uint32_t b_hi = a_lo + L::A_BYTES, b_lo = b_hi + L::B_BYTES;
    const uint32_t lane_a = (uint32_t)(g >> 2) * L::LBO_A + (uint32_t)tig * 16u + (uint32_t)(g & 3) * 4u;
    const uint32_t lane_b = (uint32_t)(g >> 2) * L::LBO_B + (uint32_t)tig * 32u + (uint32_t)(g & 3) * 4u;
    const uint32_t tmem_d = s_tmem + (uint32_t)warp * 32u;
    unsigned char* const wbuf = bw_smem + kBwdBfBytes + (size_t)warp * L::WARP_BYTES;
    unsigned char* const pa_hi = wbuf + lane_a;
    unsigned char* const pa_lo = pa_hi + L::A_BYTES;
    unsigned char* const pb_hi = wbuf + 2u * L::A_BYTES + lane_b;
    unsigned char* const pb_lo = pb_hi + L::B_BYTES;

    const unsigned rowbytes = (unsigned)b * kC * 4u;
    const size_t rowlen = (size_t)b * kC;
    const int n_ts = b / TS;
    const int tiles_per_ts = (E + NW - 1) / NW;
    const long long n_tiles = (long long)n_ts * tiles_per_ts;
    const long long per = (n_tiles + gridDim.x - 1) / gridDim.x;
    const long long lo = interleave ? (long long)blockIdx.x : (long long)blockIdx.x * per;
    const long long hi = interleave ? n_tiles : (lo + per < n_tiles ? lo + per : n_tiles);
    const long long step = interleave ? (long long)gridDim.x : 1;
    const int fq = warp & 3, fidx = warp >> 2, fnq = (NW - fq + 3) / 4;
    float* fdst = ws + ((size_t)blockIdx.x * 3 + fidx) * kDW + fq * kC * kC + (16 * ((lane >> 2) & 1) + 4 * (lane & 3) + (lane >> 3));
    for (int i = threadIdx.x; i < 3 * kDW; i += NW * 32) ws[(size_t)blockIdx.x * 3 * kDW + i] = 0.f;
    uint32_t phase = 0;
    bool pending = false, fresh = true;
    int it = 0;
    for (long long tile = lo; tile < hi; tile += step, ++it) {
        const int ts = (int)(tile / tiles_per_ts);
        const int e0 = (int)(tile - (long long)ts * tiles_per_ts) * NW + warp, t0 = ts * TS;
        if (e0 < E) {
        float2 hv[2][NT];
#pragma unroll
        for (int r = 0; r < 2; ++r) {
            int e, t;
            slab_row<kC, TS>(r, e0, t0, e, t);
            const float* src = Hin + (size_t)e * rowlen + (size_t)t * kC + 2 * tig;
#pragma unroll
            for (int nt = 0; nt < NT; ++nt) hv[r][nt] = *reinterpret_cast<const float2*>(src + nt * 8);
        }
        u64 acc[3][G::NL][2];
        slab_gather<kC, TS, DEPTH>(Gd, rowbytes, mptr, ment, E, b, e0, t0, acc);
        if (pending) {
            mbar_wait(&s_bar[warp], phase, err);
            phase ^= 1u;
        }
        float d[NT][4];
#pragma unroll
        for (int nt = 0; nt < NT; ++nt) d[nt][0] = d[nt][1] = d[nt][2] = d[nt][3] = 0.f;
#pragma unroll
        for (int term = 0; term < 3; ++term) {
            float fr[G::KS][4];
            slab_fragments<kC, TS>(acc[term], fr);
            if (WG) slab_mma_term<G::KS, NT>(d, fr, Bf + term * G::KS * NT * 32);
#pragma unroll
            for (int s = 0; s < G::KS; ++s)
#pragma unroll
                for (int q = 0; q < 4; ++q) {
                    uint32_t vh, vl;
                    split_tf32(fr[s][q], vh, vl);
                    const uint32_t off = (uint32_t)(q & 1) * 2u * L::LBO_A + (uint32_t)(4 * term + s) * L::SBO_A + (uint32_t)(q >> 1) * 64u;
                    *reinterpret_cast<uint32_t*>(pa_hi + off) = vh;
                    *reinterpret_cast<uint32_t*>(pa_lo + off) = vl;
                }
        }
#pragma unroll
        for (int r = 0; r < 2; ++r)
#pragma unroll
            for (int nt = 0; nt < NT; ++nt) {
                uint32_t xh, xl, yh, yl;
                split_tf32(hv[r][nt].x, xh, xl);
                split_tf32(hv[r][nt].y, yh, yl);
                const uint32_t off = (uint32_t)r * 2u * L::LBO_B + (uint32_t)nt * L::SBO_B;
                *reinterpret_cast<uint32_t*>(pb_hi + off) = xh;
                *reinterpret_cast<uint32_t*>(pb_lo + off) = xl;
                *reinterpret_cast<uint32_t*>(pb_hi + off + 16u) = yh;
                *reinterpret_cast<uint32_t*>(pb_lo + off + 16u) = yl;
            }
        asm volatile("fence.proxy.async.shared::cta;" ::: "memory");
        __syncwarp();
        if (lane == 0) {
            tc_fence_after();
#pragma unroll
            for (int ks = 0; ks < 2; ++ks) {
                const uint64_t dah = umma_desc2(a_hi + (uint32_t)ks * 2u * L::LBO_A, L::LBO_A, L::SBO_A);
                const uint64_t dal = umma_desc2(a_lo + (uint32_t)ks * 2u * L::LBO_A, L::LBO_A, L::SBO_A);
                const uint64_t dbh = umma_desc2(b_hi + (uint32_t)ks * 2u * L::LBO_B, L::LBO_B, L::SBO_B);
                const uint64_t dbl = umma_desc2(b_lo + (uint32_t)ks * 2u * L::LBO_B, L::LBO_B, L::SBO_B);
                umma_tf32_ss(tmem_d, dal, dbh, (!fresh || ks > 0) ? 1u : 0u);
                umma_tf32_ss(tmem_d, dah, dbl, 1u);
                umma_tf32_ss(tmem_d, dah, dbh, 1u);
            }
            umma_commit(&s_bar[warp]);
        }
        __syncwarp();
        pending = true;
        fresh = false;
        if (WG) {
#pragma unroll
            for (int r = 0; r < 2; ++r) {
                int e, t;
                slab_row<kC, TS>(r, e0, t0, e, t);
                float* dst = Gprev + (size_t)e * rowlen + (size_t)t * kC + 2 * tig;
#pragma unroll
                for (int nt = 0; nt < NT; ++nt)
                    *reinterpret_cast<float2*>(dst + nt * 8) =
                        make_float2(d[nt][2 * r] * umma_dact<ACT>(hv[r][nt].x), d[nt][2 * r + 1] * umma_dact<ACT>(hv[r][nt].y));
            }
        }
        }
        if (it % kFlushTiles == kFlushTiles - 1 || tile + step >= hi) {
            if (pending) {
                mbar_wait(&s_bar[warp], phase, err);
                phase ^= 1u;
                pending = false;
            }
            if (lane == 0) s_used[warp] = fresh ? 0 : 1;
            tc_fence_before();
            __syncthreads();
            tc_fence_after();
            if (fq < 3) {
                float sum[kC];
#pragma unroll
                for (int j = 0; j < kC; ++j) sum[j] = 0.f;
                for (int w = fidx; w < NW; w += fnq) {
                    if (!s_used[w]) continue;
                    uint32_t r[32];
                    tc_ld_32x32b_x32(s_tmem + (uint32_t)w * 32u + ((uint32_t)(32 * fq) << 16), r);
#pragma unroll
                    for (int j = 0; j < kC; ++j) sum[j] += __uint_as_float(r[j]);
                }
#pragma unroll
                for (int j = 0; j < kC; ++j) fdst[j * kC] += sum[j];
            }
            tc_fence_before();
            __syncthreads();
            tc_fence_after();
            fresh = true;
        }
    }
    if (warp == 0) asm volatile("tcgen05.dealloc.cta_group::1.sync.aligned.b32 %0, %1;" ::"r"(s_tmem), "r"(kTmemCols));
}

__global__ void __launch_bounds__(256) umma_reduce_partials_kernel(const float* __restrict__ partial, int nparts, int n,
                                                                  float* __restrict__ out, int accumulate) {
    __shared__ float red[8][32];
    const int lane = threadIdx.x & 31, slice = threadIdx.x >> 5;
    const int i = blockIdx.x * 32 + lane;
    const int per = (nparts + 7) / 8;
    const int p0 = slice * per, p1 = min(nparts, p0 + per);
    float s = 0.f;
    if (i < n)
        for (int p = p0; p < p1; ++p) s += partial[(size_t)p * n + i];
    red[slice][lane] = s;
    __syncthreads();
    if (slice == 0 && i < n) {
        float t = red[0][lane];
#pragma unroll
        for (int k = 1; k < 8; ++k) t += red[k][lane];
        out[i] = accumulate ? out[i] + t : t;
    }
}

template <int ACT, bool WG, int NW, int DEPTH>
int launch_bwd_umma(const scone_complex* cx, int b, const float* G, const float* Hin, const float* W0, const float* W1, const float* W2,
                    float* Gprev, float* ws, int* grid_out, cudaStream_t st) {
    const size_t smem = (size_t)kBwdBfBytes + (size_t)NW * BwdBuf<NW>::WARP_BYTES;
    auto kern = layer_bwd_umma_kernel<ACT, WG, NW, DEPTH>;
    static bool configured = false;
    if (!configured) {
        SCONE_CUDA(cudaFuncSetAttribute(kern, cudaFuncAttributeMaxDynamicSharedMemorySize, (int)smem));
        configured = true;
    }
    const long long n_tiles = (long long)(b / 16) * ((cx->E + NW - 1) / NW);
    const int grid = (int)(n_tiles < cx->num_sms ? n_tiles : cx->num_sms);
    *grid_out = grid;
    static int interleave = -1;
    if (interleave < 0) {
        const char* e = getenv("SCONE_UMMA_BWD_INTERLEAVE");
        interleave = (e && e[0] == '0') ? 0 : 1;
    }
    kern<<<grid, NW * 32, smem, st>>>(G, Hin, Gprev, W0, W1, W2, ws, cx->d_mptr, cx->d_ment, cx->E, b, interleave, g_umma_err);
    SCONE_LAUNCHED();
    return 0;
}

template <int ACT, bool WG>
int dispatch_bwd_umma_cfg(const scone_complex* cx, int b, const float* G, const float* Hin, const float* W0, const float* W1,
                          const float* W2, float* Gprev, float* ws, int* grid_out, cudaStream_t st) {
    static int cfg = -1;
    if (cfg < 0) {
        const char* e = getenv("SCONE_UMMA_BWD_CFG");
        cfg = e ? atoi(e) * 100 + (strchr(e, 'x') ? atoi(strchr(e, 'x') + 1) : 4) : 1204;
    }
#define SCONE_BWD_CFG(NW_, D_) \
    if (cfg == NW_ * 100 + D_) return launch_bwd_umma<ACT, WG, NW_, D_>(cx, b, G, Hin, W0, W1, W2, Gprev, ws, grid_out, st);
    SCONE_BWD_CFG(10, 4)
    SCONE_BWD_CFG(12, 4)
    SCONE_BWD_CFG(12, 6)
#undef SCONE_BWD_CFG
    scone_set_error("SCONE_UMMA_BWD_CFG: unknown configuration %d", cfg);
    return 2;
}

}

bool scone_umma_supported(const scone_complex* cx, int cin, int cout, int b) {
    return cx->d_mptr != nullptr && cin == 32 && cout == 32 && b % 16 == 0;
}

int scone_umma_forward(const scone_complex* cx, int act, int b, const float* Hin, const float* W0, const float* W1, const float* W2,
                       float* Hout, cudaStream_t st) {
    if (!g_umma_err) {
        SCONE_CUDA(cudaMalloc((void**)&g_umma_err, sizeof(int)));
        SCONE_CUDA(cudaMemset(g_umma_err, 0, sizeof(int)));
    }
    const int n_ts = (b + 15) / 16;
    const long long n_tiles = (long long)n_ts * ((cx->E + kGatherWarps - 1) / kGatherWarps);
    const int grid = (int)(n_tiles < cx->num_sms ? n_tiles : cx->num_sms);
    const int chunk = scone_dense_chunk();
    switch (act) {
        case SCONE_ACT_TANH:
            layer_fwd_umma_kernel<SCONE_ACT_TANH><<<grid, kUmmaThreads, 0, st>>>(Hin, Hout, W0, W1, W2, cx->d_mptr, cx->d_ment, cx->E, b, chunk, g_umma_err);
            break;
        case SCONE_ACT_LEAKY_RELU:
            layer_fwd_umma_kernel<SCONE_ACT_LEAKY_RELU><<<grid, kUmmaThreads, 0, st>>>(Hin, Hout, W0, W1, W2, cx->d_mptr, cx->d_ment, cx->E, b, chunk, g_umma_err);
            break;
        case SCONE_ACT_RELU:
            layer_fwd_umma_kernel<SCONE_ACT_RELU><<<grid, kUmmaThreads, 0, st>>>(Hin, Hout, W0, W1, W2, cx->d_mptr, cx->d_ment, cx->E, b, chunk, g_umma_err);
            break;
        default:
            scone_set_error("unknown activation %d", act);
            return 2;
    }
    SCONE_LAUNCHED();
    return 0;
}

int scone_umma_backward(const scone_complex* cx, int act, int b, const float* G, const float* Hin, const float* W0, const float* W1,
                        const float* W2, float* Gprev, float* dW, int accumulate, float* ws, cudaStream_t st) {
    if (!g_umma_err) {
        SCONE_CUDA(cudaMalloc((void**)&g_umma_err, sizeof(int)));
        SCONE_CUDA(cudaMemset(g_umma_err, 0, sizeof(int)));
    }
    int rc = 2, grid = 0;
#define SCONE_UMMA_BWD(A)                                                                                                      \
    case A:                                                                                                                    \
        rc = Gprev ? dispatch_bwd_umma_cfg<A, true>(cx, b, G, Hin, W0, W1, W2, Gprev, ws, &grid, st)                            \
                   : dispatch_bwd_umma_cfg<A, false>(cx, b, G, Hin, W0, W1, W2, Gprev, ws, &grid, st);                          \
        break;
    switch (act) {
        SCONE_UMMA_BWD(SCONE_ACT_TANH)
        SCONE_UMMA_BWD(SCONE_ACT_LEAKY_RELU)
        SCONE_UMMA_BWD(SCONE_ACT_RELU)
        default:
            scone_set_error("unknown activation %d", act);
            return 2;
    }
#undef SCONE_UMMA_BWD
    if (rc) return rc;
    umma_reduce_partials_kernel<<<(kDW + 31) / 32, 256, 0, st>>>(ws, 3 * grid, kDW, dW, accumulate);
    SCONE_LAUNCHED();
    return 0;
}

extern "C" int scone_set_dense_chunk(int32_t tiles) {
    SCONE_REQUIRE(tiles >= 0, "scone_set_dense_chunk: tiles per chunk must be >= 0 (0 = contiguous tile ranges per CTA)");
    g_dense_chunk = tiles;
    return 0;
}

int scone_umma_check(cudaStream_t st) {
    if (!g_umma_err) return 0;
    int e = 0;
    SCONE_CUDA(cudaMemcpyAsync(&e, g_umma_err, sizeof(int), cudaMemcpyDeviceToHost, st));
    SCONE_CUDA(cudaStreamSynchronize(st));
    if (e) {
        cudaMemset(g_umma_err, 0, sizeof(int));
        scone_set_error("layer_fwd_umma_kernel: an mbarrier wait timed out (tcgen05 protocol error); results of that launch are invalid");
        return 3;
    }
    return 0;
}
```

Before: 7.438 million.

## Run two independent trajectory groups per block with pre-split TF32 weights

Restructures the fused trajectory kernel so each block holds two 256-thread groups. Each group works through its own trajectory slots using named barriers and its own shared-memory region, while both share one copy of the weights. Layer weights are split into TF32 hi/lo pairs once at load time, so the inner MMA loop no longer re-splits them, at the cost of doubling weight shared memory. Staging capacity SE is raised, and per-trajectory row counts now go through atomics instead of local counters. The tcgen05 helpers are moved into a shared header.

Measured after the change: 7.492 million, median of 6. Within noise of the previous version (+0.7%).

```diff
diff --git a/__graft_entry__.py b/__graft_entry__.py
--- a/__graft_entry__.py
+++ b/__graft_entry__.py
@@ -23,8 +23,10 @@
 
 def build(force=False):
     os.chdir(ROOT)
-    deps = SRC + ['include/scone_b200.h', 'scone_gcn_b200/csrc/common.cuh', 'scone_gcn_b200/csrc/slab_common.cuh', 'scone_gcn_b200/csrc/fused.cuh']
-    hdrs = ['include/scone_b200.h', 'scone_gcn_b200/csrc/common.cuh', 'scone_gcn_b200/csrc/slab_common.cuh', 'scone_gcn_b200/csrc/fused.cuh']
+    deps = SRC + ['include/scone_b200.h', 'scone_gcn_b200/csrc/common.cuh', 'scone_gcn_b200/csrc/slab_common.cuh', 'scone_gcn_b200/csrc/fused.cuh',
+            'scone_gcn_b200/csrc/tcgen05.cuh']
+    hdrs = ['include/scone_b200.h', 'scone_gcn_b200/csrc/common.cuh', 'scone_gcn_b200/csrc/slab_common.cuh', 'scone_gcn_b200/csrc/fused.cuh',
+            'scone_gcn_b200/csrc/tcgen05.cuh']
     if force or _stale(OUT, deps):
         nvcc = shutil.which('nvcc') or '/usr/local/cuda/bin/nvcc'
         os.makedirs(OBJ_DIR, exist_ok=True)
diff --git a/scone_gcn_b200/csrc/scone_fused.cu b/scone_gcn_b200/csrc/scone_fused.cu
--- a/scone_gcn_b200/csrc/scone_fused.cu
+++ b/scone_gcn_b200/csrc/scone_fused.cu
@@ -9,6 +9,7 @@
 #include "slab_common.cuh"
 
 constexpr int kTrajThreads = 256;
+constexpr int kTrajGroups = 2;
 constexpr int kFuMaxD = SCONE_MAX_DEGREE;
 constexpr uint32_t kNoRow = 0xFFFFu;
 constexpr uint32_t kFlaggedKey = 0xFFFFFFu;
@@ -409,13 +410,18 @@
     unsigned long long* rows_done;
 };
 
+__device__ __forceinline__ int fu_tid() { return (int)(threadIdx.x % kTrajThreads); }
+__device__ __forceinline__ void fu_sync() {
+    asm volatile("bar.sync %0, %1;" ::"r"(1 + (int)(threadIdx.x / kTrajThreads)), "r"(kTrajThreads) : "memory");
+}
+
 template <int C>
 struct FuGeom {
     static constexpr int LDH = C + 8;
     static constexpr int LDA = 3 * C + 4;
-    static constexpr int LDW = C + 8;
+    static constexpr int LDW = C + 4;
     static constexpr int CH = 80;
-    static constexpr int SE = 1024;
+    static constexpr int SE = 1536;
     static constexpr int SP = 200;
     static constexpr int SL1 = 384;
     static constexpr int LPR = C / 4;
@@ -429,7 +435,7 @@
 template <int C>
 __device__ __forceinline__ void fu_gather(float* __restrict__ tile, const float* src, const int* ptr, const int2* ent, int pbase, int nr) {
     using G = FuGeom<C>;
-    const int lr = threadIdx.x % G::LPR, rr = threadIdx.x / G::LPR;
+    const int lr = fu_tid() % G::LPR, rr = fu_tid() / G::LPR;
     const int npad = (nr + 15) & ~15;
     for (int r = rr; r < npad; r += kTrajThreads / G::LPR) {
         u64 s0a = 0ull, s0b = 0ull, s1a = 0ull, s1b = 0ull;
@@ -472,8 +478,8 @@
     if (n_rows + 1 > G::SP || tot > G::SE) return false;
     const int* gptr = reinterpret_cast<const int*>(arena + off);
     const int2* gent = reinterpret_cast<const int2*>(gptr + align2(n_rows + 1));
-    for (int i = threadIdx.x; i <= n_rows; i += kTrajThreads) cp_async_4(sptr + i, gptr + i);
-    for (int i = threadIdx.x; i < tot; i += kTrajThreads) cp_async_8(sent + i, gent + i);
+    for (int i = fu_tid(); i <= n_rows; i += kTrajThreads) cp_async_4(sptr + i, gptr + i);
+    for (int i = fu_tid(); i < tot; i += kTrajThreads) cp_async_8(sent + i, gent + i);
     return true;
 }
 
@@ -482,22 +488,22 @@
                                         int2* sent, bool* staged) {
     using G = FuGeom<C>;
     int nr = min(G::CH, n_rows - r0);
-    for (int i = threadIdx.x; i <= nr; i += kTrajThreads) sptr[i] = __ldg(gptr + r0 + i);
-    __syncthreads();
+    for (int i = fu_tid(); i <= nr; i += kTrajThreads) sptr[i] = __ldg(gptr + r0 + i);
+    fu_sync();
     const int pbase = sptr[0];
     while (nr > 16 && sptr[nr] - pbase > G::SE) nr -= 16;
     const int cnt = sptr[nr] - pbase;
     *staged = cnt <= G::SE;
     if (*staged)
-        for (int i = threadIdx.x; i < cnt; i += kTrajThreads) sent[i] = __ldg(gent + pbase + i);
-    __syncthreads();
+        for (int i = fu_tid(); i < cnt; i += kTrajThreads) sent[i] = __ldg(gent + pbase + i);
+    fu_sync();
     return nr;
 }
 
 template <int C, bool TRANSPOSED, typename Epi>
-__device__ __forceinline__ void fu_product(const float* __restrict__ tile, const float* __restrict__ Wsm, int nr, Epi epi) {
+__device__ __forceinline__ void fu_product(const float* __restrict__ tile, const uint2* __restrict__ Ws, int nr, Epi epi) {
     using G = FuGeom<C>;
-    const int lane = threadIdx.x & 31, warp = threadIdx.x >> 5, g = lane >> 2, tig = lane & 3;
+    const int lane = fu_tid() & 31, warp = fu_tid() >> 5, g = lane >> 2, tig = lane & 3;
     const int n_mt = (nr + 15) >> 4;
     for (int tl = warp; tl < n_mt * G::NP; tl += kTrajThreads / 32) {
         const int mt = tl / G::NP, np = tl % G::NP;
@@ -508,7 +514,7 @@
             for (int q = 0; q < 4; ++q) d[j][q] = dx[j][q] = 0.f;
         const float* arow0 = tile + (size_t)(16 * mt + g) * G::LDA + tig;
         const float* arow1 = arow0 + 8 * G::LDA;
-#pragma unroll 4
+#pragma unroll 2
         for (int ks = 0; ks < 3 * C / 8; ++ks) {
             const int k0 = 8 * ks;
             uint32_t ahi[4], alo[4];
@@ -519,21 +525,18 @@
 #pragma unroll
             for (int j = 0; j < 2; ++j) {
                 const int n0 = (2 * np + j) * 8;
-                float b0, b1;
+                uint2 b0, b1;
                 if (!TRANSPOSED) {
-                    b0 = Wsm[(k0 + tig) * G::LDW + n0 + g];
-                    b1 = Wsm[(k0 + tig + 4) * G::LDW + n0 + g];
+                    b0 = Ws[(k0 + tig) * G::LDW + n0 + g];
+                    b1 = Ws[(k0 + tig + 4) * G::LDW + n0 + g];
                 } else {
                     const int term = k0 / C, co = k0 % C + tig;
-                    b0 = Wsm[(term * C + n0 + g) * G::LDW + co];
-                    b1 = Wsm[(term * C + n0 + g) * G::LDW + co + 4];
+                    b0 = Ws[(term * C + n0 + g) * G::LDW + co];
+                    b1 = Ws[(term * C + n0 + g) * G::LDW + co + 4];
                 }
-                uint32_t bh0, bl0, bh1, bl1;
-                split_tf32(b0, bh0, bl0);
-                split_tf32(b1, bh1, bl1);
-                mma_tf32(dx[j], alo, bh0, bh1);
-                mma_tf32(dx[j], ahi, bl0, bl1);
-                mma_tf32(d[j], ahi, bh0, bh1);
+                mma_tf32(dx[j], alo, b0.x, b1.x);
+                mma_tf32(dx[j], ahi, b0.y, b1.y);
+                mma_tf32(d[j], ahi, b0.x, b1.x);
             }
         }
 #pragma unroll
@@ -553,7 +556,7 @@
 template <int C>
 __device__ __forceinline__ void fu_dw(float (&acc)[FuGeom<C>::TPW][4], const float* hprev, const float* __restrict__ tile, int nr) {
     using G = FuGeom<C>;
-    const int lane = threadIdx.x & 31, warp = threadIdx.x >> 5, g = lane >> 2, tig = lane & 3;
+    const int lane = fu_tid() & 31, warp = fu_tid() >> 5, g = lane >> 2, tig = lane & 3;
     const int mt = warp % G::NMT, ntg = warp / G::NMT;
     for (int k0 = 0; k0 < nr; k0 += 8) {
         const int ra = k0 + tig, rb = ra + 4;
@@ -579,31 +582,41 @@
     }
 }
 
+template <int C>
+__host__ __device__ constexpr size_t fu_group_floats(int D, int cap_rows) {
+    using G = FuGeom<C>;
+    return (size_t)G::CH * G::LDA + (size_t)D * C + 2 * ((D + 3) & ~3) + 2 * (size_t)G::SE + G::SP + 2 * G::SL1 + (size_t)cap_rows * G::LDH;
+}
+
 template <int C, int ACT, bool GRAD, bool BIG>
-__global__ void __launch_bounds__(kTrajThreads, 2) fused_traj_kernel(const TrajArgs a) {
+__global__ void __launch_bounds__(kTrajGroups * kTrajThreads, 1) fused_traj_kernel(const TrajArgs a) {
     using G = FuGeom<C>;
     extern __shared__ __align__(16) unsigned char sm[];
     const int L = a.L, D = a.D;
-    float* Wsm = reinterpret_cast<float*>(sm);
-    float* w1s = Wsm + (size_t)(kFusedMaxL - 1) * 3 * C * G::LDW;
+    uint2* Wst = reinterpret_cast<uint2*>(sm);
+    float* w1s = reinterpret_cast<float*>(Wst + (size_t)(kFusedMaxL - 1) * 3 * C * G::LDW);
     float* wos = w1s + 3 * C;
-    float* tile = wos + C;
-    float* zs = tile + (size_t)G::CH * G::LDA;
+    const int grp = (int)(threadIdx.x / kTrajThreads);
+    float* tile = wos + C + (size_t)grp * fu_group_floats<C>(D, BIG ? 0 : a.cap_rows);
+    int2* sent = reinterpret_cast<int2*>(tile + (size_t)G::CH * G::LDA);
+    int* sptr = reinterpret_cast<int*>(sent + G::SE);
+    float* l1s = reinterpret_cast<float*>(sptr + G::SP);
+    float* zs = l1s + 2 * G::SL1;
     float* lg = zs + (size_t)D * C;
     float* dl = lg + ((D + 3) & ~3);
-    int2* sent = reinterpret_cast<int2*>(dl + ((D + 3) & ~3));
-    int* sptr = reinterpret_cast<int*>(sent + G::SE);
-    float* l1s = reinterpret_cast<float*>(sptr + G::SP);
-    float* rows_sm = l1s + 2 * G::SL1;
-    const int tid = threadIdx.x, lane = tid & 31, warp = tid >> 5;
+    float* rows_sm = dl + ((D + 3) & ~3);
+    const int tid = fu_tid(), lane = tid & 31, warp = tid >> 5;
+    auto slot = [&]() { return kTrajGroups * (int)blockIdx.x + (int)(threadIdx.x / kTrajThreads); };
 
     for (int l = 2; l <= L; ++l)
-        for (int i = tid; i < 3 * C * C; i += kTrajThreads) {
+        for (int i = threadIdx.x; i < 3 * C * C; i += kTrajGroups * kTrajThreads) {
             const int term = i / (C * C), rem = i % (C * C);
-            Wsm[(size_t)(l - 2) * 3 * C * G::LDW + (term * C + rem / C) * G::LDW + rem % C] = a.W[a.w_off[3 * (l - 1) + term] + rem];
-        }
-    for (int i = tid; i < 3 * C; i += kTrajThreads) w1s[i] = a.W[a.w_off[i / C] + i % C];
-    for (int i = tid; i < C; i += kTrajThreads) wos[i] = a.W[a.w_off[3 * L] + i];
+            uint2 w;
+            split_tf32(a.W[a.w_off[3 * (l - 1) + term] + rem], w.x, w.y);
+            Wst[(size_t)(l - 2) * 3 * C * G::LDW + (term * C + rem / C) * G::LDW + rem % C] = w;
+        }
+    for (int i = threadIdx.x; i < 3 * C; i += kTrajGroups * kTrajThreads) w1s[i] = a.W[a.w_off[i / C] + i % C];
+    for (int i = threadIdx.x; i < C; i += kTrajGroups * kTrajThreads) wos[i] = a.W[a.w_off[3 * L] + i];
     __syncthreads();
 
     float acc[kFusedMaxL - 1][G::TPW][4];
@@ -613,13 +626,19 @@
         for (int s = 0; s < G::TPW; ++s)
 #pragma unroll
             for (int q = 0; q < 4; ++q) acc[l][s][q] = 0.f;
-    float acc1 = 0.f, acc_out = 0.f, acc_nll = 0.f, acc_cnt = 0.f;
-    unsigned long long n_fwd = 0, n_bwd = 0;
-
-    float* rows = BIG ? a.scratch + (size_t)blockIdx.x * a.scratch_stride : rows_sm;
-
-    __shared__ int s_range[2];
-    __shared__ int s_hdr[2][kFusedHdrW];
+    float acc1 = 0.f, acc_out = 0.f;
+    __shared__ float s_nll[kTrajGroups][32], s_cnt[kTrajGroups];
+    if (warp == 0) {
+        s_nll[grp][lane] = 0.f;
+        if (lane == 0) s_cnt[grp] = 0.f;
+    }
+
+    float* rows = BIG ? a.scratch + (size_t)slot() * a.scratch_stride : rows_sm;
+
+    __shared__ int s_ranges[kTrajGroups][2];
+    __shared__ int s_hdrs[kTrajGroups][2][kFusedHdrW];
+    int* s_range = s_ranges[grp];
+    int (*s_hdr)[kFusedHdrW] = s_hdrs[grp];
     if (tid == 0) {
         int f = 0, hi = a.b;
         while (f < hi) {
@@ -637,9 +656,12 @@
         s_range[0] = BIG ? f : lo;
         s_range[1] = BIG ? lo : a.b;
     }
-    __syncthreads();
+    fu_sync();
     const int i_lo = s_range[0], i_hi = s_range[1];
-    auto index_of = [&](int kk) { return i_lo + kk * (int)gridDim.x + ((kk & 1) ? (int)gridDim.x - 1 - (int)blockIdx.x : (int)blockIdx.x); };
+    auto index_of = [&](int kk) {
+        const int n_slots = kTrajGroups * (int)gridDim.x;
+        return i_lo + kk * n_slots + ((kk & 1) ? n_slots - 1 - slot() : slot());
+    };
     auto issue_first = [&](const int* hn, float* l1buf) -> bool {
         const int n1 = hn[1];
         if (3 * n1 <= G::SL1) {
@@ -655,7 +677,7 @@
         t = a.order[index_of(0)];
         const int rid = a.rows != nullptr ? a.rows[t] : t;
         if (tid < kFusedHdrW) s_hdr[0][tid] = a.hdr[(size_t)rid * kFusedHdrW + tid];
-        __syncthreads();
+        fu_sync();
         pf_first = issue_first(s_hdr[0], l1s);
     }
     for (int k = 0; have; ++k) {
@@ -665,7 +687,7 @@
         const int t_next = have_next ? a.order[index_of(k + 1)] : 0;
         bool issued_next = false, pf_first_next = false;
         cp_async_wait_all();
-        __syncthreads();
+        fu_sync();
         int n[kFusedMaxL + 1], hb[kFusedMaxL + 2];
         int tot = 0;
         n[0] = 0;
@@ -677,7 +699,10 @@
             tot += n[l];
         }
         const float* l1 = reinterpret_cast<const float*>(a.arena + (unsigned)h[4]);
-        n_fwd += (unsigned long long)tot;
+        if (a.rows_done != nullptr && tid == 0) {
+            atomicAdd(a.rows_done, (unsigned long long)tot);
+            if (GRAD) atomicAdd(a.rows_done + 1, (unsigned long long)hb[L]);
+        }
         const int tot_f[kFusedMaxL + 1] = {0, 0, h[12], h[14]};
         const int tot_b[kFusedMaxL + 1] = {0, 0, h[15] & 0xFFFF, (int)((unsigned)h[15] >> 16)};
         bool pf = pf_first;
@@ -689,7 +714,7 @@
             rows[(size_t)r * G::LDH + c] = fu_act<ACT>(z);
         }
         const int rid_next = have_next ? (a.rows != nullptr ? a.rows[t_next] : t_next) : 0;
-        __syncthreads();
+        fu_sync();
 #pragma unroll
         for (int l = 2; l <= kFusedMaxL; ++l) {
             if (l > L) break;
@@ -698,7 +723,7 @@
             const int2* ent = reinterpret_cast<const int2*>(ptr + align2(nl + 1));
             const float* hprev = rows + (size_t)hb[l - 1] * G::LDH;
             float* hout = rows + (size_t)hb[l] * G::LDH;
-            const float* Wl = Wsm + (size_t)(l - 2) * 3 * C * G::LDW;
+            const uint2* Wl = Wst + (size_t)(l - 2) * 3 * C * G::LDW;
             bool pf_next = false;
             if (nl == 0)
                 pf_next = l < L ? fu_prefetch<C>(a.arena, (unsigned)h[5 + (l - 1)], n[l + 1], tot_f[l < kFusedMaxL ? l + 1 : l], sptr, sent)
@@ -714,7 +739,7 @@
                     if (staged) fu_gather<C>(tile, hprev, sptr, sent, sptr[0], nr);
                     else fu_gather<C>(tile, hprev, sptr, ent, 0, nr);
                 }
-                __syncthreads();
+                fu_sync();
                 if (r0 + nr >= nl)
                     pf_next = l < L ? fu_prefetch<C>(a.arena, (unsigned)h[5 + (l - 1)], n[l + 1], tot_f[l < kFusedMaxL ? l + 1 : l], sptr, sent)
                                     : fu_prefetch<C>(a.arena, (unsigned)h[9], D, h[10], sptr, sent);
@@ -723,12 +748,12 @@
                     *reinterpret_cast<float2*>(o) = make_float2(fu_act<ACT>(v0), fu_act<ACT>(v1));
                 });
                 cp_async_wait_all();
-                __syncthreads();
+                fu_sync();
                 r0 += nr;
             }
             if (nl == 0) {
                 cp_async_wait_all();
-                __syncthreads();
+                fu_sync();
             }
             pf = pf_next;
         }
@@ -741,7 +766,7 @@
         } else if (h[10] <= G::SE) {
             for (int i = tid; i <= D; i += kTrajThreads) sptr[i] = __ldg(rptr + i);
             for (int i = tid; i < h[10]; i += kTrajThreads) sent[i] = __ldg(rent + i);
-            __syncthreads();
+            fu_sync();
             rptr = sptr;
             rent = sent;
         }
@@ -760,7 +785,7 @@
             for (int o = 16; o > 0; o >>= 1) part += __shfl_xor_sync(0xffffffffu, part, o);
             if (lane == 0) lg[j] = part;
         }
-        __syncthreads();
+        fu_sync();
         if (warp == 0) {
             float mx = -3.4e38f;
             for (int j = lane; j < D; j += 32) mx = fmaxf(mx, lg[j]);
@@ -778,14 +803,14 @@
                 if (a.logprobs != nullptr) a.logprobs[(size_t)t * D + j] = lp;
                 if (GRAD) {
                     dl[j] = mk * (expf(lp) - (j == y ? 1.f : 0.f));
-                    if (j == y) acc_nll += -mk * lp;
+                    if (j == y) s_nll[grp][lane] += -mk * lp;
                 }
             }
-            if (GRAD && lane == 0) acc_cnt += mk;
+            if (GRAD && lane == 0) s_cnt[grp] += mk;
         }
         if (!GRAD) {
             cp_async_wait_all();
-            __syncthreads();
+            fu_sync();
             if (have_next) pf_first = issue_first(s_hdr[(k + 1) & 1], l1s + ((k + 1) & 1) * G::SL1);
             t = t_next;
             have = have_next;
@@ -794,7 +819,7 @@
         const int nL = n[L];
         float* gL = rows + (size_t)hb[L] * G::LDH;
         for (int r = tid; r < nL; r += kTrajThreads) gL[(size_t)r * G::LDH + C] = 0.f;
-        __syncthreads();
+        fu_sync();
         if (tid < C) {
             float s = acc_out;
             for (int j = 0; j < D; ++j) s = fmaf(dl[j], zs[j * C + tid], s);
@@ -808,14 +833,14 @@
                 if (r != kNoRow) atomicAdd(&gL[(size_t)r * G::LDH + C], __int_as_float(en.y) * dl[((uint32_t)en.x >> 16) & 0x7FFFu]);
             }
         }
-        __syncthreads();
+        fu_sync();
         pf = L >= 2 ? fu_prefetch<C>(a.arena, (unsigned)h[7 + (L - 2)], n[L - 1], tot_b[L], sptr, sent) : false;
         for (int i = tid; i < nL * C; i += kTrajThreads) {
             const int r = i / C, c = i % C;
             gL[(size_t)r * G::LDH + c] = gL[(size_t)r * G::LDH + C] * wos[c] * fu_dact<ACT>(hL[(size_t)r * G::LDH + c]);
         }
         cp_async_wait_all();
-        __syncthreads();
+        fu_sync();
 #pragma unroll
         for (int l = kFusedMaxL; l >= 2; --l) {
             if (l > L) continue;
@@ -825,8 +850,7 @@
             const float* gl = rows + (size_t)hb[l] * G::LDH;
             float* hprev = rows + (size_t)hb[l - 1] * G::LDH;
             float* gprev = hprev;
-            const float* Wl = Wsm + (size_t)(l - 2) * 3 * C * G::LDW;
-            n_bwd += (unsigned long long)np_;
+            const uint2* Wl = Wst + (size_t)(l - 2) * 3 * C * G::LDW;
             bool pf_next = false;
             if (np_ == 0 && l > 2) pf_next = fu_prefetch<C>(a.arena, (unsigned)h[7 + (l - 3)], n[l - 2], tot_b[l - 1], sptr, sent);
             for (int r0 = 0; r0 < np_;) {
@@ -840,7 +864,7 @@
                     if (staged) fu_gather<C>(tile, gl, sptr, sent, sptr[0], nr);
                     else fu_gather<C>(tile, gl, sptr, ent, 0, nr);
                 }
-                __syncthreads();
+                fu_sync();
                 if (r0 + nr >= np_) {
                     if (l > 2) {
                         pf_next = fu_prefetch<C>(a.arena, (unsigned)h[7 + (l - 3)], n[l - 2], tot_b[l - 1], sptr, sent);
@@ -850,19 +874,19 @@
                     }
                 }
                 fu_dw<C>(acc[l - 2], hprev + (size_t)r0 * G::LDH, tile, nr);
-                __syncthreads();
+                fu_sync();
                 fu_product<C, true>(tile, Wl, nr, [&](int r, int col, float v0, float v1) {
                     const float2 hv = *reinterpret_cast<const float2*>(hprev + (size_t)(r0 + r) * G::LDH + col);
                     *reinterpret_cast<float2*>(gprev + (size_t)(r0 + r) * G::LDH + col) =
                         make_float2(v0 * fu_dact<ACT>(hv.x), v1 * fu_dact<ACT>(hv.y));
                 });
                 cp_async_wait_all();
-                __syncthreads();
+                fu_sync();
                 r0 += nr;
             }
             if (np_ == 0) {
                 cp_async_wait_all();
-                __syncthreads();
+                fu_sync();
             }
             pf = pf_next;
         }
@@ -875,7 +899,7 @@
         }
         if (have_next && !issued_next) {
             cp_async_wait_all();
-            __syncthreads();
+            fu_sync();
             pf_first_next = issue_first(s_hdr[(k + 1) & 1], l1s + ((k + 1) & 1) * G::SL1);
         }
         pf_first = pf_first_next;
@@ -883,41 +907,38 @@
         have = have_next;
     }
 
-    if (a.rows_done != nullptr && tid == 0 && (n_fwd | n_bwd)) {
-        atomicAdd(a.rows_done, n_fwd);
-        atomicAdd(a.rows_done + 1, n_bwd);
-    }
-    if (!GRAD) return;
-    float* P = a.partial + (size_t)blockIdx.x * (a.n_params + 2);
-    if (tid < 3 * C) P[a.w_off[tid / C] + tid % C] = acc1;
-    {
-        const int g = lane >> 2, tig = lane & 3;
-        const int mt = warp % G::NMT, ntg = warp / G::NMT;
-#pragma unroll
-        for (int l = 2; l <= kFusedMaxL; ++l) {
-            if (l > L) break;
-#pragma unroll
-            for (int s = 0; s < G::TPW; ++s) {
-                const int nt = ntg + G::WPM * s;
-                if (nt >= G::NNT) continue;
-                const int nn = 8 * nt + 2 * tig, term = nn / C, co = nn % C;
-                float* dst = P + a.w_off[3 * (l - 1) + term];
-                const int ci = 16 * mt + g;
-                dst[ci * C + co] = acc[l - 2][s][0];
-                dst[ci * C + co + 1] = acc[l - 2][s][1];
-                dst[(ci + 8) * C + co] = acc[l - 2][s][2];
-                dst[(ci + 8) * C + co + 1] = acc[l - 2][s][3];
-            }
-        }
-    }
-    if (tid < C) P[a.w_off[3 * L] + tid] = acc_out;
-    if (warp == 0) {
-        float s = acc_nll;
-#pragma unroll
-        for (int o = 16; o > 0; o >>= 1) s += __shfl_xor_sync(0xffffffffu, s, o);
-        if (lane == 0) {
-            P[a.n_params] = s;
-            P[a.n_params + 1] = acc_cnt;
+    if (GRAD) {
+        float* P = a.partial + (size_t)slot() * (a.n_params + 2);
+        if (tid < 3 * C) P[a.w_off[tid / C] + tid % C] = acc1;
+        {
+            const int g = lane >> 2, tig = lane & 3;
+            const int mt = warp % G::NMT, ntg = warp / G::NMT;
+#pragma unroll
+            for (int l = 2; l <= kFusedMaxL; ++l) {
+                if (l > L) break;
+#pragma unroll
+                for (int s = 0; s < G::TPW; ++s) {
+                    const int nt = ntg + G::WPM * s;
+                    if (nt >= G::NNT) continue;
+                    const int nn = 8 * nt + 2 * tig, term = nn / C, co = nn % C;
+                    float* dst = P + a.w_off[3 * (l - 1) + term];
+                    const int ci = 16 * mt + g;
+                    dst[ci * C + co] = acc[l - 2][s][0];
+                    dst[ci * C + co + 1] = acc[l - 2][s][1];
+                    dst[(ci + 8) * C + co] = acc[l - 2][s][2];
+                    dst[(ci + 8) * C + co + 1] = acc[l - 2][s][3];
+                }
+            }
+        }
+        if (tid < C) P[a.w_off[3 * L] + tid] = acc_out;
+        if (warp == 0) {
+            float s = s_nll[grp][lane];
+#pragma unroll
+            for (int o = 16; o > 0; o >>= 1) s += __shfl_xor_sync(0xffffffffu, s, o);
+            if (lane == 0) {
+                P[a.n_params] = s;
+                P[a.n_params + 1] = s_cnt[grp];
+            }
         }
     }
 }
@@ -953,8 +974,7 @@
 template <int C>
 size_t traj_smem_bytes(int D, int cap_rows) {
     using G = FuGeom<C>;
-    size_t fl = (size_t)(kFusedMaxL - 1) * 3 * C * G::LDW + 3 * C + C + (size_t)G::CH * G::LDA + (size_t)D * C + 2 * ((D + 3) & ~3) +
-                2 * (size_t)G::SE + G::SP + 2 * G::SL1 + (size_t)cap_rows * G::LDH;
+    const size_t fl = (size_t)(kFusedMaxL - 1) * 3 * C * G::LDW * 2 + 3 * C + C + kTrajGroups * fu_group_floats<C>(D, cap_rows);
     return fl * sizeof(float);
 }
 
@@ -967,11 +987,11 @@
         configured = true;
     }
     TrajArgs a = base;
-    fused_traj_kernel<C, ACT, GRAD, false><<<grid_small, kTrajThreads, smem_small, st>>>(a);
+    fused_traj_kernel<C, ACT, GRAD, false><<<grid_small / kTrajGroups, kTrajGroups * kTrajThreads, smem_small, st>>>(a);
     SCONE_LAUNCHED();
     if (grid_big > 0) {
         if (GRAD) a.partial = base.partial + (size_t)grid_small * (base.n_params + 2);
-        fused_traj_kernel<C, ACT, GRAD, true><<<grid_big, kTrajThreads, smem_big, st>>>(a);
+        fused_traj_kernel<C, ACT, GRAD, true><<<grid_big / kTrajGroups, kTrajGroups * kTrajThreads, smem_big, st>>>(a);
         SCONE_LAUNCHED();
     }
     return 0;
@@ -1122,14 +1142,15 @@
     f->big_rows = L * f->bound_list;
     f->traj_smem_small = C == 32 ? traj_smem_bytes<32>(cx->D, f->cap_rows) : traj_smem_bytes<16>(cx->D, f->cap_rows);
     f->traj_smem_big = C == 32 ? traj_smem_bytes<32>(cx->D, 0) : traj_smem_bytes<16>(cx->D, 0);
-    if (f->traj_smem_small > 113 * 1024) {
-        const size_t over = f->traj_smem_small - 113 * 1024;
-        const int less = (int)((over + ldh * 4 - 1) / (ldh * 4));
+    constexpr size_t kTrajSmemMax = 227 * 1024 - 1024;
+    if (f->traj_smem_small > kTrajSmemMax) {
+        const size_t over = f->traj_smem_small - kTrajSmemMax;
+        const int less = (int)((over + kTrajGroups * ldh * 4 - 1) / (kTrajGroups * ldh * 4));
         f->cap_rows = f->cap_rows > less + 32 ? f->cap_rows - less : 32;
         f->traj_smem_small = C == 32 ? traj_smem_bytes<32>(cx->D, f->cap_rows) : traj_smem_bytes<16>(cx->D, f->cap_rows);
     }
-    f->grid_small = 2 * cx->num_sms;
-    f->grid_big = f->big_rows > f->cap_rows ? 2 * cx->num_sms : 0;
+    f->grid_small = kTrajGroups * cx->num_sms;
+    f->grid_big = f->big_rows > f->cap_rows ? kTrajGroups * cx->num_sms : 0;
     if (f->grid_big) {
         f->scratch_stride = (size_t)f->big_rows * ldh;
         SCONE_CUDA(cudaMalloc((void**)&f->d_scratch, (size_t)f->grid_big * f->scratch_stride * sizeof(float)));
diff --git a/scone_gcn_b200/csrc/scone_umma.cu b/scone_gcn_b200/csrc/scone_umma.cu
--- a/scone_gcn_b200/csrc/scone_umma.cu
+++ b/scone_gcn_b200/csrc/scone_umma.cu
@@ -5,69 +5,15 @@
 namespace {
 
 #include "slab_common.cuh"
+#include "tcgen05.cuh"
 
 constexpr int kGatherWarps = 16, kGroupWarps = 8, kUmmaThreads = kGatherWarps * 32;
 constexpr int kC = 32;
 constexpr int kGatherDepth = 4;
 constexpr uint32_t kTmemCols = 512;
 constexpr uint32_t kColsAhi = 0, kColsAlo = 96, kColsD = 192, kColsGroup = 224;
-constexpr uint32_t kIdesc = (1u << 4) | (2u << 7) | (2u << 10) | ((32u >> 3) << 17) | ((128u >> 4) << 24);
+constexpr uint32_t kIdesc = umma_idesc_tf32(32, false);
 constexpr uint32_t kLbo = 512, kSbo = 128;
-constexpr int kSpinLimit = 4000000;
-
-__device__ __forceinline__ uint32_t smem_u32(const void* p) { return (uint32_t)__cvta_generic_to_shared(p); }
-__device__ __forceinline__ void tc_fence_before() { asm volatile("tcgen05.fence::before_thread_sync;" ::: "memory"); }
-__device__ __forceinline__ void tc_fence_after() { asm volatile("tcgen05.fence::after_thread_sync;" ::: "memory"); }
-__device__ __forceinline__ void tc_st_16x128b_x2(uint32_t taddr, uint32_t r0, uint32_t r1, uint32_t r2, uint32_t r3) {
-    asm volatile("tcgen05.st.sync.aligned.16x128b.x2.b32 [%0], {%1, %2, %3, %4};" ::"r"(taddr), "r"(r0), "r"(r1), "r"(r2), "r"(r3) : "memory");
-}
-__device__ __forceinline__ void tc_ld_16x256b_x4(uint32_t taddr, float (&d)[4][4]) {
-    uint32_t r[16];
-    asm volatile("tcgen05.ld.sync.aligned.16x256b.x4.b32 {%0, %1, %2, %3, %4, %5, %6, %7, %8, %9, %10, %11, %12, %13, %14, %15}, [%16];"
-                 : "=r"(r[0]), "=r"(r[1]), "=r"(r[2]), "=r"(r[3]), "=r"(r[4]), "=r"(r[5]), "=r"(r[6]), "=r"(r[7]), "=r"(r[8]), "=r"(r[9]),
-                   "=r"(r[10]), "=r"(r[11]), "=r"(r[12]), "=r"(r[13]), "=r"(r[14]), "=r"(r[15])
-                 : "r"(taddr)
-                 : "memory");
-    asm volatile("tcgen05.wait::ld.sync.aligned;" ::: "memory");
-#pragma unroll
-    for (int nt = 0; nt < 4; ++nt)
-#pragma unroll
-        for (int q = 0; q < 4; ++q) d[nt][q] = __uint_as_float(r[4 * nt + q]);
-}
-__device__ __forceinline__ void mbar_init(uint64_t* bar, uint32_t count) {
-    asm volatile("mbarrier.init.shared::cta.b64 [%0], %1;" ::"r"(smem_u32(bar)), "r"(count));
-}
-__device__ __forceinline__ bool mbar_try_wait(uint64_t* bar, uint32_t parity) {
-    uint32_t ok;
-    asm volatile("{\n\t.reg .pred p;\n\tmbarrier.try_wait.parity.shared::cta.b64 p, [%1], %2;\n\tselp.b32 %0, 1, 0, p;\n\t}"
-                 : "=r"(ok)
-                 : "r"(smem_u32(bar)), "r"(parity)
-                 : "memory");
-    return ok != 0;
-}
-__device__ __forceinline__ void mbar_wait(uint64_t* bar, uint32_t parity, int* err) {
-    int spins = 0;
-    while (!mbar_try_wait(bar, parity)) {
-        if (++spins > kSpinLimit) {
-            *err = 1;
-            break;
-        }
-    }
-}
-__device__ __forceinline__ void umma_commit(uint64_t* bar) {
-    asm volatile("tcgen05.commit.cta_group::1.mbarrier::arrive::one.shared::cluster.b64 [%0];" ::"r"(smem_u32(bar)) : "memory");
-}
-__device__ __forceinline__ void umma_tf32_ts(uint32_t tmem_d, uint32_t tmem_a, uint64_t desc_b, uint32_t accumulate) {
-    asm volatile(
-        "{\n\t.reg .pred p;\n\tsetp.ne.b32 p, %4, 0;\n\t"
-        "tcgen05.mma.cta_group::1.kind::tf32 [%0], [%1], %2, %3, {%5, %5, %5, %5}, p;\n\t}"
-        ::"r"(tmem_d), "r"(tmem_a), "l"(desc_b), "r"(kIdesc), "r"(accumulate), "r"(0u)
-        : "memory");
-}
-__device__ __forceinline__ uint64_t umma_desc(uint32_t saddr) {
-    return (uint64_t)((saddr >> 4) & 0x3FFF) | ((uint64_t)((kLbo >> 4) & 0x3FFF) << 16) | ((uint64_t)((kSbo >> 4) & 0x3FFF) << 32) |
-           ((uint64_t)1 << 46);
-}
 
 template <int ACT>
 __global__ void __launch_bounds__(kUmmaThreads, 1) layer_fwd_umma_kernel(const float* __restrict__ Hin, float* __restrict__ Hout,
@@ -192,10 +138,10 @@
                         const uint32_t bhi = smem_u32(&Bs[0][0]), blo = smem_u32(&Bs[1][0]);
 #pragma unroll
                         for (int j = 0; j < 12; ++j) {
-                            const uint64_t dh = umma_desc(bhi + (uint32_t)j * 2 * kLbo), dl = umma_desc(blo + (uint32_t)j * 2 * kLbo);
-                            umma_tf32_ts(tbase + kColsD, tbase + kColsAlo + 8 * j, dh, j > 0 ? 1u : 0u);
-                            umma_tf32_ts(tbase + kColsD, tbase + kColsAhi + 8 * j, dl, 1u);
-                            umma_tf32_ts(tbase + kColsD, tbase + kColsAhi + 8 * j, dh, 1u);
+                            const uint64_t dh = umma_desc(bhi + (uint32_t)j * 2 * kLbo, kLbo, kSbo), dl = umma_desc(blo + (uint32_t)j * 2 * kLbo, kLbo, kSbo);
+                            umma_tf32_ts(tbase + kColsD, tbase + kColsAlo + 8 * j, dh, kIdesc, j > 0 ? 1u : 0u);
+                            umma_tf32_ts(tbase + kColsD, tbase + kColsAhi + 8 * j, dl, kIdesc, 1u);
+                            umma_tf32_ts(tbase + kColsD, tbase + kColsAhi + 8 * j, dh, kIdesc, 1u);
                         }
                         umma_commit(&s_dfull[group]);
                     }
@@ -242,30 +188,6 @@
     static constexpr uint32_t WARP_BYTES = 2u * A_BYTES + 2u * B_BYTES;
 };
 constexpr uint32_t kBwdBfBytes = 3u * 4u * 4u * 32u * 16u;
-
-__device__ __forceinline__ uint64_t umma_desc2(uint32_t saddr, uint32_t lbo, uint32_t sbo) {
-    return (uint64_t)((saddr >> 4) & 0x3FFF) | ((uint64_t)((lbo >> 4) & 0x3FFF) << 16) | ((uint64_t)((sbo >> 4) & 0x3FFF) << 32) |
-           ((uint64_t)1 << 46);
-}
-__device__ __forceinline__ void umma_tf32_ss(uint32_t tmem_d, uint64_t desc_a, uint64_t desc_b, uint32_t accumulate) {
-    asm volatile(
-        "{\n\t.reg .pred p;\n\tsetp.ne.b32 p, %4, 0;\n\t"
-        "tcgen05.mma.cta_group::1.kind::tf32 [%0], %1, %2, %3, {%5, %5, %5, %5}, p;\n\t}"
-        ::"r"(tmem_d), "l"(desc_a), "l"(desc_b), "r"(kIdesc), "r"(accumulate), "r"(0u)
-        : "memory");
-}
-__device__ __forceinline__ void tc_ld_32x32b_x32(uint32_t taddr, uint32_t (&r)[32]) {
-    asm volatile(
-        "tcgen05.ld.sync.aligned.32x32b.x32.b32 {%0, %1, %2, %3, %4, %5, %6, %7, %8, %9, %10, %11, %12, %13, %14, %15, %16, %17, %18, "
-        "%19, %20, %21, %22, %23, %24, %25, %26, %27, %28, %29, %30, %31}, [%32];"
-        : "=r"(r[0]), "=r"(r[1]), "=r"(r[2]), "=r"(r[3]), "=r"(r[4]), "=r"(r[5]), "=r"(r[6]), "=r"(r[7]), "=r"(r[8]), "=r"(r[9]),
-          "=r"(r[10]), "=r"(r[11]), "=r"(r[12]), "=r"(r[13]), "=r"(r[14]), "=r"(r[15]), "=r"(r[16]), "=r"(r[17]), "=r"(r[18]),
-          "=r"(r[19]), "=r"(r[20]), "=r"(r[21]), "=r"(r[22]), "=r"(r[23]), "=r"(r[24]), "=r"(r[25]), "=r"(r[26]), "=r"(r[27]),
-          "=r"(r[28]), "=r"(r[29]), "=r"(r[30]), "=r"(r[31])
-        : "r"(taddr)
-        : "memory");
-    asm volatile("tcgen05.wait::ld.sync.aligned;" ::: "memory");
-}
 
 template <int ACT>
 __device__ __forceinline__ float umma_dact(float h) {
@@ -388,13 +310,13 @@
             tc_fence_after();
 #pragma unroll
             for (int ks = 0; ks < 2; ++ks) {
-                const uint64_t dah = umma_desc2(a_hi + (uint32_t)ks * 2u * L::LBO_A, L::LBO_A, L::SBO_A);
-                const uint64_t dal = umma_desc2(a_lo + (uint32_t)ks * 2u * L::LBO_A, L::LBO_A, L::SBO_A);
-                const uint64_t dbh = umma_desc2(b_hi + (uint32_t)ks * 2u * L::LBO_B, L::LBO_B, L::SBO_B);
-                const uint64_t dbl = umma_desc2(b_lo + (uint32_t)ks * 2u * L::LBO_B, L::LBO_B, L::SBO_B);
-                umma_tf32_ss(tmem_d, dal, dbh, (!fresh || ks > 0) ? 1u : 0u);
-                umma_tf32_ss(tmem_d, dah, dbl, 1u);
-                umma_tf32_ss(tmem_d, dah, dbh, 1u);
+                const uint64_t dah = umma_desc(a_hi + (uint32_t)ks * 2u * L::LBO_A, L::LBO_A, L::SBO_A);
+                const uint64_t dal = umma_desc(a_lo + (uint32_t)ks * 2u * L::LBO_A, L::LBO_A, L::SBO_A);
+                const uint64_t dbh = umma_desc(b_hi + (uint32_t)ks * 2u * L::LBO_B, L::LBO_B, L::SBO_B);
+                const uint64_t dbl = umma_desc(b_lo + (uint32_t)ks * 2u * L::LBO_B, L::LBO_B, L::SBO_B);
+                umma_tf32_ss(tmem_d, dal, dbh, kIdesc, (!fresh || ks > 0) ? 1u : 0u);
+                umma_tf32_ss(tmem_d, dah, dbl, kIdesc, 1u);
+                umma_tf32_ss(tmem_d, dah, dbh, kIdesc, 1u);
             }
             umma_commit(&s_bar[warp]);
         }
diff --git a/scone_gcn_b200/csrc/tcgen05.cuh b/scone_gcn_b200/csrc/tcgen05.cuh
--- /dev/null
+++ b/scone_gcn_b200/csrc/tcgen05.cuh
@@ -0,0 +1,97 @@
+#pragma once
+#include <stdint.h>
+
+constexpr int kSpinLimit = 4000000;
+
+__host__ __device__ constexpr uint32_t umma_idesc_tf32(uint32_t n, bool b_mn_major) {
+    return (1u << 4) | (2u << 7) | (2u << 10) | ((b_mn_major ? 1u : 0u) << 16) | ((n >> 3) << 17) | ((128u >> 4) << 24);
+}
+
+__device__ __forceinline__ uint32_t smem_u32(const void* p) { return (uint32_t)__cvta_generic_to_shared(p); }
+__device__ __forceinline__ void tc_fence_before() { asm volatile("tcgen05.fence::before_thread_sync;" ::: "memory"); }
+__device__ __forceinline__ void tc_fence_after() { asm volatile("tcgen05.fence::after_thread_sync;" ::: "memory"); }
+__device__ __forceinline__ void tc_st_16x128b_x2(uint32_t taddr, uint32_t r0, uint32_t r1, uint32_t r2, uint32_t r3) {
+    asm volatile("tcgen05.st.sync.aligned.16x128b.x2.b32 [%0], {%1, %2, %3, %4};" ::"r"(taddr), "r"(r0), "r"(r1), "r"(r2), "r"(r3) : "memory");
+}
+__device__ __forceinline__ void tc_st_32x32b_x8(uint32_t taddr, const uint32_t (&r)[8]) {
+    asm volatile("tcgen05.st.sync.aligned.32x32b.x8.b32 [%0], {%1, %2, %3, %4, %5, %6, %7, %8};"
+                 ::"r"(taddr), "r"(r[0]), "r"(r[1]), "r"(r[2]), "r"(r[3]), "r"(r[4]), "r"(r[5]), "r"(r[6]), "r"(r[7])
+                 : "memory");
+}
+__device__ __forceinline__ void tc_wait_st() { asm volatile("tcgen05.wait::st.sync.aligned;" ::: "memory"); }
+__device__ __forceinline__ void tc_ld_16x256b_x4(uint32_t taddr, float (&d)[4][4]) {
+    uint32_t r[16];
+    asm volatile("tcgen05.ld.sync.aligned.16x256b.x4.b32 {%0, %1, %2, %3, %4, %5, %6, %7, %8, %9, %10, %11, %12, %13, %14, %15}, [%16];"
+                 : "=r"(r[0]), "=r"(r[1]), "=r"(r[2]), "=r"(r[3]), "=r"(r[4]), "=r"(r[5]), "=r"(r[6]), "=r"(r[7]), "=r"(r[8]), "=r"(r[9]),
+                   "=r"(r[10]), "=r"(r[11]), "=r"(r[12]), "=r"(r[13]), "=r"(r[14]), "=r"(r[15])
+                 : "r"(taddr)
+                 : "memory");
+    asm volatile("tcgen05.wait::ld.sync.aligned;" ::: "memory");
+#pragma unroll
+    for (int nt = 0; nt < 4; ++nt)
+#pragma unroll
+        for (int q = 0; q < 4; ++q) d[nt][q] = __uint_as_float(r[4 * nt + q]);
+}
+__device__ __forceinline__ void tc_ld_32x32b_x8(uint32_t taddr, float (&d)[8]) {
+    uint32_t r[8];
+    asm volatile("tcgen05.ld.sync.aligned.32x32b.x8.b32 {%0, %1, %2, %3, %4, %5, %6, %7}, [%8];"
+                 : "=r"(r[0]), "=r"(r[1]), "=r"(r[2]), "=r"(r[3]), "=r"(r[4]), "=r"(r[5]), "=r"(r[6]), "=r"(r[7])
+                 : "r"(taddr)
+                 : "memory");
+    asm volatile("tcgen05.wait::ld.sync.aligned;" ::: "memory");
+#pragma unroll
+    for (int q = 0; q < 8; ++q) d[q] = __uint_as_float(r[q]);
+}
+__device__ __forceinline__ void tc_ld_32x32b_x32(uint32_t taddr, uint32_t (&r)[32]) {
+    asm volatile(
+        "tcgen05.ld.sync.aligned.32x32b.x32.b32 {%0, %1, %2, %3, %4, %5, %6, %7, %8, %9, %10, %11, %12, %13, %14, %15, %16, %17, %18, "
+        "%19, %20, %21, %22, %23, %24, %25, %26, %27, %28, %29, %30, %31}, [%32];"
+        : "=r"(r[0]), "=r"(r[1]), "=r"(r[2]), "=r"(r[3]), "=r"(r[4]), "=r"(r[5]), "=r"(r[6]), "=r"(r[7]), "=r"(r[8]), "=r"(r[9]),
+          "=r"(r[10]), "=r"(r[11]), "=r"(r[12]), "=r"(r[13]), "=r"(r[14]), "=r"(r[15]), "=r"(r[16]), "=r"(r[17]), "=r"(r[18]),
+          "=r"(r[19]), "=r"(r[20]), "=r"(r[21]), "=r"(r[22]), "=r"(r[23]), "=r"(r[24]), "=r"(r[25]), "=r"(r[26]), "=r"(r[27]),
+          "=r"(r[28]), "=r"(r[29]), "=r"(r[30]), "=r"(r[31])
+        : "r"(taddr)
+        : "memory");
+    asm volatile("tcgen05.wait::ld.sync.aligned;" ::: "memory");
+}
+__device__ __forceinline__ void mbar_init(uint64_t* bar, uint32_t count) {
+    asm volatile("mbarrier.init.shared::cta.b64 [%0], %1;" ::"r"(smem_u32(bar)), "r"(count));
+}
+__device__ __forceinline__ bool mbar_try_wait(uint64_t* bar, uint32_t parity) {
+    uint32_t ok;
+    asm volatile("{\n\t.reg .pred p;\n\tmbarrier.try_wait.parity.shared::cta.b64 p, [%1], %2;\n\tselp.b32 %0, 1, 0, p;\n\t}"
+                 : "=r"(ok)
+                 : "r"(smem_u32(bar)), "r"(parity)
+                 : "memory");
+    return ok != 0;
+}
+__device__ __forceinline__ void mbar_wait(uint64_t* bar, uint32_t parity, int* err) {
+    int spins = 0;
+    while (!mbar_try_wait(bar, parity)) {
+        if (++spins > kSpinLimit) {
+            *err = 1;
+            break;
+        }
+    }
+}
+__device__ __forceinline__ void umma_commit(uint64_t* bar) {
+    asm volatile("tcgen05.commit.cta_group::1.mbarrier::arrive::one.shared::cluster.b64 [%0];" ::"r"(smem_u32(bar)) : "memory");
+}
+__device__ __forceinline__ void umma_tf32_ts(uint32_t tmem_d, uint32_t tmem_a, uint64_t desc_b, uint32_t idesc, uint32_t accumulate) {
+    asm volatile(
+        "{\n\t.reg .pred p;\n\tsetp.ne.b32 p, %4, 0;\n\t"
+        "tcgen05.mma.cta_group::1.kind::tf32 [%0], [%1], %2, %3, {%5, %5, %5, %5}, p;\n\t}"
+        ::"r"(tmem_d), "r"(tmem_a), "l"(desc_b), "r"(idesc), "r"(accumulate), "r"(0u)
+        : "memory");
+}
+__device__ __forceinline__ void umma_tf32_ss(uint32_t tmem_d, uint64_t desc_a, uint64_t desc_b, uint32_t idesc, uint32_t accumulate) {
+    asm volatile(
+        "{\n\t.reg .pred p;\n\tsetp.ne.b32 p, %4, 0;\n\t"
+        "tcgen05.mma.cta_group::1.kind::tf32 [%0], %1, %2, %3, {%5, %5, %5, %5}, p;\n\t}"
+        ::"r"(tmem_d), "l"(desc_a), "l"(desc_b), "r"(idesc), "r"(accumulate), "r"(0u)
+        : "memory");
+}
+__device__ __forceinline__ uint64_t umma_desc(uint32_t saddr, uint32_t lbo, uint32_t sbo) {
+    return (uint64_t)((saddr >> 4) & 0x3FFF) | ((uint64_t)((lbo >> 4) & 0x3FFF) << 16) | ((uint64_t)((sbo >> 4) & 0x3FFF) << 32) |
+           ((uint64_t)1 << 46);
+}
```
